# CarloLucibello/GraphNeuralNetworks.jl

Hardware: NVIDIA H100
Metric: edges/sec fwd+bwd GCNConv 128-dim on 100M-edge graph (higher is better)
Workload: dtype f32

## Files before the change

graphneuralnetworks.jl_b200/csrc/dense_tc.cu:

```cuda
#include "common.cuh"
#include <map>

namespace gnnb {

namespace tc {
constexpr int BM = 128;
constexpr int BK = 32;
constexpr int BN = 128;
constexpr int NSTAGE = 3;
constexpr int PRODUCERS = 128;
constexpr int CONSUMER_WARPS = 8;
constexpr int THREADS = PRODUCERS + CONSUMER_WARPS * 32;
constexpr int KBLK_BYTES = BM * 128;
constexpr int W_BYTES = 4 * KBLK_BYTES;
constexpr int SMEM_W_BIG = 0;
constexpr int SMEM_W_SMALL = W_BYTES;
constexpr int SMEM_A = 2 * W_BYTES;
constexpr int SMEM_BIAS = SMEM_A + NSTAGE * 2 * KBLK_BYTES;
constexpr int SMEM_BAR = SMEM_BIAS + 512;
constexpr int SMEM_TOTAL = SMEM_BAR + 64;

__device__ __forceinline__ uint32_t s_u32(const void* p) { return (uint32_t)__cvta_generic_to_shared(p); }
__device__ __forceinline__ void bar_init(uint32_t bar, uint32_t count) {
    asm volatile("mbarrier.init.shared::cta.b64 [%0], %1;" ::"r"(bar), "r"(count) : "memory");
}
__device__ __forceinline__ void bar_arrive(uint32_t bar) {
    asm volatile("mbarrier.arrive.shared::cta.b64 _, [%0];" ::"r"(bar) : "memory");
}
__device__ __forceinline__ bool bar_try(uint32_t bar, uint32_t parity) {
    uint32_t ok;
    asm volatile("{\n\t.reg .pred p;\n\tmbarrier.try_wait.parity.shared::cta.b64 p, [%1], %2;\n\tselp.u32 %0, 1, 0, p;\n\t}"
                 : "=r"(ok) : "r"(bar), "r"(parity) : "memory");
    return ok != 0;
}
__device__ __forceinline__ bool bar_wait(uint32_t bar, uint32_t parity, int* err) {
    for (uint32_t spin = 0; spin < (1u << 26); ++spin) {
        if (bar_try(bar, parity)) return true;
        if ((spin & 1023) == 1023 && *(volatile int*)err) return false;
    }
    atomicExch(err, 1);
    return false;
}
__device__ __forceinline__ float tf32_big(float x) { return __uint_as_float(__float_as_uint(x) & 0xffffe000u); }
__device__ __forceinline__ float tf32_small(float x, float b) { return isinf(x) ? 0.f : x - b; }
__device__ __forceinline__ float4 tf32_small(float4 v, float4 b) {
    return make_float4(tf32_small(v.x, b.x), tf32_small(v.y, b.y), tf32_small(v.z, b.z), tf32_small(v.w, b.w));
}
__device__ __forceinline__ void fence_proxy_async() { asm volatile("fence.proxy.async.shared::cta;" ::: "memory"); }
__device__ __forceinline__ void prefetch_l2(const void* p, uint32_t bytes) {
    asm volatile("cp.async.bulk.prefetch.L2.global [%0], %1;" ::"l"(p), "r"(bytes) : "memory");
}

__device__ __forceinline__ uint64_t gmma_desc(uint32_t saddr) {
    return (uint64_t)((saddr & 0x3ffffu) >> 4) | ((uint64_t)1 << 16) | ((uint64_t)(1024 >> 4) << 32) | ((uint64_t)1 << 62);
}
__device__ __forceinline__ void wgmma_tf32(float* d, uint64_t da, uint64_t db, uint32_t accumulate) {
    asm volatile(
        "{\n\t.reg .pred p;\n\tsetp.ne.b32 p, %66, 0;\n\t"
        "wgmma.mma_async.sync.aligned.m64n128k8.f32.tf32.tf32 "
        "{%0, %1, %2, %3, %4, %5, %6, %7, %8, %9, %10, %11, %12, %13, %14, %15, %16, %17, %18, %19, %20, %21, %22, %23, "
        "%24, %25, %26, %27, %28, %29, %30, %31, %32, %33, %34, %35, %36, %37, %38, %39, %40, %41, %42, %43, %44, %45, %46, "
        "%47, %48, %49, %50, %51, %52, %53, %54, %55, %56, %57, %58, %59, %60, %61, %62, %63}, %64, %65, p, 1, 1;\n\t}"
        : "+f"(d[0]), "+f"(d[1]), "+f"(d[2]), "+f"(d[3]), "+f"(d[4]), "+f"(d[5]), "+f"(d[6]), "+f"(d[7]), "+f"(d[8]),
          "+f"(d[9]), "+f"(d[10]), "+f"(d[11]), "+f"(d[12]), "+f"(d[13]), "+f"(d[14]), "+f"(d[15]), "+f"(d[16]),
          "+f"(d[17]), "+f"(d[18]), "+f"(d[19]), "+f"(d[20]), "+f"(d[21]), "+f"(d[22]), "+f"(d[23]), "+f"(d[24]),
          "+f"(d[25]), "+f"(d[26]), "+f"(d[27]), "+f"(d[28]), "+f"(d[29]), "+f"(d[30]), "+f"(d[31]), "+f"(d[32]),
          "+f"(d[33]), "+f"(d[34]), "+f"(d[35]), "+f"(d[36]), "+f"(d[37]), "+f"(d[38]), "+f"(d[39]), "+f"(d[40]),
          "+f"(d[41]), "+f"(d[42]), "+f"(d[43]), "+f"(d[44]), "+f"(d[45]), "+f"(d[46]), "+f"(d[47]), "+f"(d[48]),
          "+f"(d[49]), "+f"(d[50]), "+f"(d[51]), "+f"(d[52]), "+f"(d[53]), "+f"(d[54]), "+f"(d[55]), "+f"(d[56]),
          "+f"(d[57]), "+f"(d[58]), "+f"(d[59]), "+f"(d[60]), "+f"(d[61]), "+f"(d[62]), "+f"(d[63])
        : "l"(da), "l"(db), "r"(accumulate));
}
__device__ __forceinline__ void fence_acc(float* d) {
#pragma unroll
    for (int i = 0; i < 64; ++i) asm volatile("" : "+f"(d[i])::"memory");
}
__device__ __forceinline__ void wgmma_fence() { asm volatile("wgmma.fence.sync.aligned;" ::: "memory"); }
__device__ __forceinline__ void wgmma_commit() { asm volatile("wgmma.commit_group.sync.aligned;" ::: "memory"); }
__device__ __forceinline__ void wgmma_wait_all() { asm volatile("wgmma.wait_group.sync.aligned 0;" ::: "memory"); }

__device__ __forceinline__ void mma_kblock(float* dm, float* dc, uint32_t a_big, uint32_t a_small, uint32_t b_big,
                                           uint32_t b_small, bool first) {
    wgmma_fence();
    fence_acc(dm);
    fence_acc(dc);
#pragma unroll
    for (int j = 0; j < 4; ++j) {
        const uint32_t o = j * 32;
        const uint32_t acc = (first && j == 0) ? 0u : 1u;
        wgmma_tf32(dc, gmma_desc(a_small + o), gmma_desc(b_big + o), acc);
        wgmma_tf32(dc, gmma_desc(a_big + o), gmma_desc(b_small + o), 1u);
        wgmma_tf32(dm, gmma_desc(a_big + o), gmma_desc(b_big + o), dm == dc ? 1u : acc);
    }
    wgmma_commit();
    wgmma_wait_all();
    fence_acc(dm);
    fence_acc(dc);
}

struct Params {
    const float* __restrict__ x;
    const float* __restrict__ w;
    const float* __restrict__ bias;
    const float* __restrict__ addend;
    float* __restrict__ y;
    int64_t M;
    int K, Nout, relu, ldw;
    int* err;
    const float* __restrict__ wimg;
    const float* __restrict__ act;
    float* __restrict__ colsum;
    uint32_t* __restrict__ mask;
};


template <bool MASK = false>
__device__ __forceinline__ void store_tile(const Params& p, const float* dm, const float* dc, const float* sbias, int64_t row0,
                                           int col_base, int ncols) {
    const int lane = threadIdx.x & 31, w4 = (threadIdx.x >> 5) & 3;
    const int64_t r0 = row0 + w4 * 16 + (lane >> 2);
    uint32_t mw[2] = {0u, 0u};
#pragma unroll
    for (int j = 0; j < BN / 8; ++j) {
        const int c = 8 * j + 2 * (lane & 3);
        if (c >= ncols) continue;
        const float b0 = sbias[col_base + c], b1 = sbias[col_base + c + 1];
#pragma unroll
        for (int h = 0; h < 2; ++h) {
            const int64_t row = r0 + 8 * h;
            if (row >= p.M) continue;
            float2 o = make_float2((dm[4 * j + 2 * h] + dc[4 * j + 2 * h]) + b0, (dm[4 * j + 2 * h + 1] + dc[4 * j + 2 * h + 1]) + b1);
            const size_t at = (size_t)row * p.Nout + col_base + c;
            if (p.addend) {
                const float2 a = *reinterpret_cast<const float2*>(p.addend + at);
                o.x += a.x; o.y += a.y;
            }
            if (p.relu) { o.x = fmax_nan(o.x, 0.f); o.y = fmax_nan(o.y, 0.f); }
            *reinterpret_cast<float2*>(p.y + at) = o;
            if (MASK) mw[h] |= ((uint32_t)(o.x > 0.f) << (2 * j)) | ((uint32_t)(o.y > 0.f) << (2 * j + 1));
        }
    }
    if (MASK) {
#pragma unroll
        for (int h = 0; h < 2; ++h) {
            const int64_t row = r0 + 8 * h;
            if (row < p.M) p.mask[(size_t)row * 4 + (lane & 3)] = mw[h];
        }
    }
}

template <bool MASK = false>
__device__ __forceinline__ void consume_tiles(const Params& p, uint32_t sbase, const float* sbias, int KB, int64_t ntiles) {
    const int warp = threadIdx.x >> 5, lane = threadIdx.x & 31;
    const uint32_t bar_full = sbase + SMEM_BAR, bar_empty = bar_full + 8 * NSTAGE;
    const int wg = (warp - PRODUCERS / 32) >> 2;
    float dm[64] = {}, dc[64] = {};
    uint32_t it = 0;
    bool alive = true;
    for (int64_t tile = blockIdx.x; alive && tile < ntiles; tile += gridDim.x) {
        for (int kb = 0; kb < KB; ++kb, ++it) {
            const int stage = it % NSTAGE;
            if (!bar_wait(bar_full + 8 * stage, (it / NSTAGE) & 1, p.err)) { alive = false; break; }
            const uint32_t a_big = sbase + SMEM_A + stage * 2 * KBLK_BYTES + wg * 64 * 128, a_small = a_big + KBLK_BYTES;
            const uint32_t w_big = sbase + SMEM_W_BIG + kb * KBLK_BYTES, w_small = sbase + SMEM_W_SMALL + kb * KBLK_BYTES;
            mma_kblock(dm, dc, a_big, a_small, w_big, w_small, kb == 0);
            if (lane == 0) bar_arrive(bar_empty + 8 * stage);
        }
        if (alive) store_tile<MASK>(p, dm, dc, sbias, tile * BM + wg * 64, 0, p.Nout);
    }
}

template <bool MASK>
__device__ __forceinline__ void linear_body(const Params& p) {
    extern __shared__ __align__(1024) unsigned char smem[];
    const int tid = threadIdx.x, warp = tid >> 5;
    const int KB = p.K / BK;
    const int64_t ntiles = (p.M + BM - 1) / BM;
    const uint32_t sbase = s_u32(smem);
    const uint32_t bar_full = sbase + SMEM_BAR;
    const uint32_t bar_empty = bar_full + 8 * NSTAGE;
    float* sbias = reinterpret_cast<float*>(smem + SMEM_BIAS);

    if (tid == 0) {
        for (int s = 0; s < NSTAGE; ++s) { bar_init(bar_full + 8 * s, PRODUCERS); bar_init(bar_empty + 8 * s, CONSUMER_WARPS); }
        asm volatile("fence.mbarrier_init.release.cluster;" ::: "memory");
    }
    for (int i = tid; i < BN; i += THREADS) sbias[i] = (p.bias && i < p.Nout) ? p.bias[i] : 0.f;
    {
        const int kv = p.K >> 2;
        for (int idx = tid; idx < BN * kv; idx += THREADS) {
            const int n = idx / kv, c4 = idx - n * kv, kb = c4 >> 3, c = c4 & 7;
            const float4 v = n < p.Nout ? __ldg(reinterpret_cast<const float4*>(p.w + (size_t)n * p.ldw) + c4)
                                        : make_float4(0.f, 0.f, 0.f, 0.f);
            const float4 b = make_float4(tf32_big(v.x), tf32_big(v.y), tf32_big(v.z), tf32_big(v.w));
            const float4 s = tf32_small(v, b);
            const int off = kb * KBLK_BYTES + (n >> 3) * 1024 + (n & 7) * 128 + ((c ^ (n & 7)) << 4);
            *reinterpret_cast<float4*>(smem + SMEM_W_BIG + off) = b;
            *reinterpret_cast<float4*>(smem + SMEM_W_SMALL + off) = s;
        }
    }
    fence_proxy_async();
    __syncthreads();

    if (warp < PRODUCERS / 32) {
        const int c = tid & 7, r16 = tid >> 3, rr = r16 & 7;
        const int64_t my_tiles = (ntiles > (int64_t)blockIdx.x) ? (ntiles - blockIdx.x + gridDim.x - 1) / gridDim.x : 0;
        const int64_t total = my_tiles * KB;
        auto fetch = [&](int64_t item, float4* v) {
            const int64_t tile = blockIdx.x + (item / KB) * gridDim.x;
            const int kb = (int)(item % KB);
#pragma unroll
            for (int i = 0; i < 8; ++i) {
                const int64_t row = tile * BM + r16 + 16 * i;
                v[i] = (item < total && row < p.M)
                           ? __ldg(reinterpret_cast<const float4*>(p.x + (size_t)row * p.K + kb * BK) + c)
                           : make_float4(0.f, 0.f, 0.f, 0.f);
            }
        };
        float4 v[8], vn[8];
        fetch(0, v);
        for (int64_t it = 0; it < total; ++it) {
            fetch(it + 1, vn);
            const int stage = (int)(it % NSTAGE);
            if (!bar_wait(bar_empty + 8 * stage, (uint32_t)(((it / NSTAGE) & 1) ^ 1), p.err)) break;
            unsigned char* abig = smem + SMEM_A + stage * 2 * KBLK_BYTES;
#pragma unroll
            for (int i = 0; i < 8; ++i) {
                const float4 b = make_float4(tf32_big(v[i].x), tf32_big(v[i].y), tf32_big(v[i].z), tf32_big(v[i].w));
                const float4 s = tf32_small(v[i], b);
                const int off = ((r16 >> 3) + 2 * i) * 1024 + rr * 128 + ((c ^ rr) << 4);
                *reinterpret_cast<float4*>(abig + off) = b;
                *reinterpret_cast<float4*>(abig + KBLK_BYTES + off) = s;
            }
            fence_proxy_async();
            bar_arrive(bar_full + 8 * stage);
#pragma unroll
            for (int i = 0; i < 8; ++i) v[i] = vn[i];
        }
    } else {
        consume_tiles<MASK>(p, sbase, sbias, KB, ntiles);
    }
}

__global__ void __launch_bounds__(THREADS, 1) linear_tf32x3_kernel(const Params p) { linear_body<false>(p); }
__global__ void __launch_bounds__(THREADS, 1) linear_relu_mask_kernel(const Params p) { linear_body<true>(p); }

template <bool MASK>
__device__ __forceinline__ void bwd_dx_body(const Params& p) {
    extern __shared__ __align__(1024) unsigned char smem[];
    const int tid = threadIdx.x, warp = tid >> 5, lane = tid & 31;
    const int64_t ntiles = (p.M + BM - 1) / BM;
    const uint32_t sbase = s_u32(smem);
    const uint32_t bar_full = sbase + SMEM_BAR;
    const uint32_t bar_empty = bar_full + 8 * NSTAGE;
    float* sbias = reinterpret_cast<float*>(smem + SMEM_BIAS);

    if (tid == 0) {
        for (int s = 0; s < NSTAGE; ++s) { bar_init(bar_full + 8 * s, PRODUCERS); bar_init(bar_empty + 8 * s, CONSUMER_WARPS); }
        asm volatile("fence.mbarrier_init.release.cluster;" ::: "memory");
    }
    for (int i = tid; i < BN; i += THREADS) sbias[i] = 0.f;
    for (int idx = tid; idx < BN * 32; idx += THREADS) {
        const int n = idx >> 5, c4 = idx & 31, kb = c4 >> 3, c = c4 & 7;
        float4 v = make_float4(0.f, 0.f, 0.f, 0.f);
        if (n < p.Nout) {
            const float* col = p.w + (size_t)(4 * c4) * p.Nout + n;
            v = make_float4(__ldg(col), __ldg(col + p.Nout), __ldg(col + 2 * p.Nout), __ldg(col + 3 * p.Nout));
        }
        const float4 b = make_float4(tf32_big(v.x), tf32_big(v.y), tf32_big(v.z), tf32_big(v.w));
        const float4 s = tf32_small(v, b);
        const int off = kb * KBLK_BYTES + (n >> 3) * 1024 + (n & 7) * 128 + ((c ^ (n & 7)) << 4);
        *reinterpret_cast<float4*>(smem + SMEM_W_BIG + off) = b;
        *reinterpret_cast<float4*>(smem + SMEM_W_SMALL + off) = s;
    }
    fence_proxy_async();
    __syncthreads();

    if (warp < PRODUCERS / 32) {
        const int c = tid & 7, r16 = tid >> 3, rr = r16 & 7;
        const float4 zero = make_float4(0.f, 0.f, 0.f, 0.f);
        const int64_t my_tiles = (ntiles > (int64_t)blockIdx.x) ? (ntiles - blockIdx.x + gridDim.x - 1) / gridDim.x : 0;
        const int64_t total = my_tiles * 4;
        using MaskReg = typename std::conditional<MASK, uint2, float4>::type;
        auto fetch = [&](int64_t item, float4* g, MaskReg* m) {
            const int64_t tile = blockIdx.x + (item >> 2) * gridDim.x;
            const int kb = (int)(item & 3);
#pragma unroll
            for (int i = 0; i < 8; ++i) {
                const int64_t row = tile * BM + r16 + 16 * i;
                const bool in = item < total && row < p.M;
                const size_t at = (size_t)row * 128 + kb * BK;
                g[i] = in ? __ldg(reinterpret_cast<const float4*>(p.x + at) + c) : zero;
                if constexpr (MASK) m[i] = in ? __ldg(reinterpret_cast<const uint2*>(p.mask + (size_t)row * 4) + (c & 1)) : make_uint2(0u, 0u);
                else m[i] = (in && p.act) ? __ldg(reinterpret_cast<const float4*>(p.act + at) + c) : zero;
            }
        };
        auto masked = [&](float4* g, const MaskReg* m, int kb) {
            if constexpr (MASK) {
                const int s = 8 * kb + 2 * (c >> 1);
#pragma unroll
                for (int i = 0; i < 8; ++i) {
                    g[i].x = (m[i].x >> s) & 1u ? g[i].x : 0.f; g[i].y = (m[i].x >> (s + 1)) & 1u ? g[i].y : 0.f;
                    g[i].z = (m[i].y >> s) & 1u ? g[i].z : 0.f; g[i].w = (m[i].y >> (s + 1)) & 1u ? g[i].w : 0.f;
                }
            } else {
                if (!p.act) return;
#pragma unroll
                for (int i = 0; i < 8; ++i) {
                    g[i].x = m[i].x > 0.f ? g[i].x : 0.f; g[i].y = m[i].y > 0.f ? g[i].y : 0.f;
                    g[i].z = m[i].z > 0.f ? g[i].z : 0.f; g[i].w = m[i].w > 0.f ? g[i].w : 0.f;
                }
            }
        };
        float4 cs = zero;
        float4 g[8], gn[8];
        MaskReg mn[8];
        fetch(0, g, mn);
        masked(g, mn, 0);
        for (int64_t it = 0; it < total; ++it) {
            const int kb = (int)(it & 3);
            if (tid == 0 && kb == 0 && it + 4 < total) {
                const int64_t r0 = (blockIdx.x + ((it >> 2) + 1) * gridDim.x) * BM, nr = (p.M - r0 < BM) ? p.M - r0 : BM;
                prefetch_l2(p.x + (size_t)r0 * 128, (uint32_t)(nr * 512));
                if (!MASK && p.act) prefetch_l2(p.act + (size_t)r0 * 128, (uint32_t)(nr * 512));
            }
            fetch(it + 1, gn, mn);
            if (p.colsum) {
                float4 t = zero;
#pragma unroll
                for (int i = 0; i < 8; ++i) { t.x += g[i].x; t.y += g[i].y; t.z += g[i].z; t.w += g[i].w; }
#pragma unroll
                for (int o = 8; o <= 16; o <<= 1) {
                    t.x += __shfl_xor_sync(0xffffffffu, t.x, o); t.y += __shfl_xor_sync(0xffffffffu, t.y, o);
                    t.z += __shfl_xor_sync(0xffffffffu, t.z, o); t.w += __shfl_xor_sync(0xffffffffu, t.w, o);
                }
                if ((lane >> 3) == kb) { cs.x += t.x; cs.y += t.y; cs.z += t.z; cs.w += t.w; }
            }
            const int stage = (int)(it % NSTAGE);
            if (!bar_wait(bar_empty + 8 * stage, (uint32_t)(((it / NSTAGE) & 1) ^ 1), p.err)) break;
            unsigned char* abig = smem + SMEM_A + stage * 2 * KBLK_BYTES;
#pragma unroll
            for (int i = 0; i < 8; ++i) {
                const float4 b = make_float4(tf32_big(g[i].x), tf32_big(g[i].y), tf32_big(g[i].z), tf32_big(g[i].w));
                const float4 s = tf32_small(g[i], b);
                const int off = ((r16 >> 3) + 2 * i) * 1024 + rr * 128 + ((c ^ rr) << 4);
                *reinterpret_cast<float4*>(abig + off) = b;
                *reinterpret_cast<float4*>(abig + KBLK_BYTES + off) = s;
            }
            fence_proxy_async();
            bar_arrive(bar_full + 8 * stage);
#pragma unroll
            for (int i = 0; i < 8; ++i) g[i] = gn[i];
            masked(g, mn, (kb + 1) & 3);
        }
        if (p.colsum) reinterpret_cast<float4*>(p.colsum + ((size_t)blockIdx.x * 4 + warp) * 128 + (lane >> 3) * BK)[c] = cs;
    } else {
        consume_tiles(p, sbase, sbias, 128 / BK, ntiles);
    }
}

__global__ void __launch_bounds__(THREADS, 1) linear_bwd_dx_kernel(const Params p) { bwd_dx_body<false>(p); }
__global__ void __launch_bounds__(THREADS, 1) linear_bwd_dx_mask_kernel(const Params p) { bwd_dx_body<true>(p); }
}

namespace tcw {
using namespace tc;
constexpr int WSTAGE = 3;
constexpr int FLUSH = 4;
constexpr int STAGE_BYTES = 4 * KBLK_BYTES;
constexpr int SMEM_BARW = WSTAGE * STAGE_BYTES;
constexpr int SMEM_TOTALW = SMEM_BARW + 64;

struct ParamsW {
    const float* __restrict__ dpre;
    const float* __restrict__ x;
    float* __restrict__ partial;
    int64_t M, rows_per_cta;
    int Din;
    int* err;
    const float* __restrict__ act;
    const uint32_t* __restrict__ mask;
};
constexpr int L2_AHEAD = 3;

__device__ __forceinline__ int kmajor_off(int n, int k) {
    return (n >> 3) * 1024 + (n & 7) * 128 + ((((k >> 2) ^ (n & 7))) << 4) + (k & 3) * 4;
}

template <bool FUSED, bool MASK = false>
__device__ __forceinline__ void dw_body(const ParamsW& p) {
    extern __shared__ __align__(1024) unsigned char smem[];
    const int tid = threadIdx.x, warp = tid >> 5, lane = tid & 31;
    const uint32_t sbase = s_u32(smem);
    const uint32_t bar_full = sbase + SMEM_BARW, bar_empty = bar_full + 8 * WSTAGE;
    const int nfB = p.Din >> 2;
    const int64_t r_begin = (int64_t)blockIdx.x * p.rows_per_cta;
    const int64_t r_end = (r_begin + p.rows_per_cta < p.M) ? r_begin + p.rows_per_cta : p.M;
    const int64_t nblk = (r_end > r_begin) ? (r_end - r_begin + 31) / 32 : 0;

    if (tid == 0) {
        for (int s = 0; s < WSTAGE; ++s) { bar_init(bar_full + 8 * s, PRODUCERS); bar_init(bar_empty + 8 * s, CONSUMER_WARPS); }
        asm volatile("fence.mbarrier_init.release.cluster;" ::: "memory");
    }
    for (int i = tid; i < SMEM_BARW / 16; i += THREADS) reinterpret_cast<float4*>(smem)[i] = make_float4(0.f, 0.f, 0.f, 0.f);
    fence_proxy_async();
    __syncthreads();

    if (warp < PRODUCERS / 32) {
        const int rl = lane >> 2, fl = lane & 3;
        auto load = [&](const float* src, int ld, int nf, int64_t blk, float4* v) {
#pragma unroll
            for (int q = 0; q < 8; ++q) {
                const int64_t r = r_begin + blk * 32 + rl + 8 * (q & 3);
                const int f = 4 * (warp + 4 * (q >> 2)) + fl;
                v[q] = (blk < nblk && r < r_end && f < nf) ? __ldg(reinterpret_cast<const float4*>(src + (size_t)r * ld) + f)
                                                           : make_float4(0.f, 0.f, 0.f, 0.f);
            }
        };
        auto put1 = [&](unsigned char* big, int n, int k, float e) {
            const int off = kmajor_off(n, k);
            const float b = tf32_big(e);
            *reinterpret_cast<float*>(big + off) = b;
            *reinterpret_cast<float*>(big + KBLK_BYTES + off) = tf32_small(e, b);
        };
        auto put = [&](unsigned char* big, int n0, int k, float4 v) {
            put1(big, n0, k, v.x); put1(big, n0 + 1, k, v.y); put1(big, n0 + 2, k, v.z); put1(big, n0 + 3, k, v.w);
        };
        auto stage_in = [&](int64_t blk, const float4* va, const float4* vb) {
            const int stage = (int)(blk % WSTAGE);
            if (!bar_wait(bar_empty + 8 * stage, (uint32_t)(((blk / WSTAGE) & 1) ^ 1), p.err)) return false;
            unsigned char* st = smem + stage * STAGE_BYTES;
#pragma unroll
            for (int q = 0; q < 8; ++q) {
                const int k = rl + 8 * (q & 3);
                const int f = 4 * (warp + 4 * (q >> 2)) + fl;
                put(st, 4 * f, k, va[q]);
                if (f < nfB) put(st + 2 * KBLK_BYTES, 4 * f, k, vb[q]);
            }
            fence_proxy_async();
            bar_arrive(bar_full + 8 * stage);
            return true;
        };
        if constexpr (!FUSED) {
            float4 va[8], vb[8], na[8], nb[8];
            load(p.dpre, 128, 32, 0, va);
            load(p.x, p.Din, nfB, 0, vb);
            for (int64_t blk = 0; blk < nblk; ++blk) {
                load(p.dpre, 128, 32, blk + 1, na);
                load(p.x, p.Din, nfB, blk + 1, nb);
                if (!stage_in(blk, va, vb)) break;
#pragma unroll
                for (int q = 0; q < 8; ++q) { va[q] = na[q]; vb[q] = nb[q]; }
            }
        } else if constexpr (MASK) {
            float4 va[8], vb[8], na[8];
            uint2 nm[4];
            auto load_mask = [&](int64_t blk) {
#pragma unroll
                for (int q = 0; q < 4; ++q) {
                    const int64_t r = r_begin + blk * 32 + rl + 8 * q;
                    nm[q] = (blk < nblk && r < r_end) ? __ldg(reinterpret_cast<const uint2*>(p.mask + (size_t)r * 4) + (fl & 1))
                                                      : make_uint2(0u, 0u);
                }
            };
            auto promote = [&]() {
#pragma unroll
                for (int q = 0; q < 8; ++q) {
                    const uint2 m = nm[q & 3];
                    const int s = 4 * (warp + 4 * (q >> 2)) + 2 * (fl >> 1);
                    va[q].x = (m.x >> s) & 1u ? na[q].x : 0.f; va[q].y = (m.x >> (s + 1)) & 1u ? na[q].y : 0.f;
                    va[q].z = (m.y >> s) & 1u ? na[q].z : 0.f; va[q].w = (m.y >> (s + 1)) & 1u ? na[q].w : 0.f;
                }
            };
            load(p.dpre, 128, 32, 0, na);
            load_mask(0);
            promote();
            for (int64_t blk = 0; blk < nblk; ++blk) {
                if (tid == 0 && blk + L2_AHEAD < nblk) {
                    const int64_t ra = r_begin + 32 * (blk + L2_AHEAD), nr = (r_end - ra < 32) ? r_end - ra : 32;
                    prefetch_l2(p.dpre + (size_t)ra * 128, (uint32_t)(nr * 512));
                    prefetch_l2(p.x + (size_t)ra * p.Din, (uint32_t)(nr * p.Din * 4));
                }
                load(p.dpre, 128, 32, blk + 1, na);
                load_mask(blk + 1);
                load(p.x, p.Din, nfB, blk, vb);
                if (!stage_in(blk, va, vb)) break;
                promote();
            }
        } else {
            float4 va[8], vb[8], na[8], nm[8];
            auto promote = [&]() {
#pragma unroll
                for (int q = 0; q < 8; ++q) {
                    va[q] = na[q];
                    if (p.act) {
                        va[q].x = nm[q].x > 0.f ? va[q].x : 0.f; va[q].y = nm[q].y > 0.f ? va[q].y : 0.f;
                        va[q].z = nm[q].z > 0.f ? va[q].z : 0.f; va[q].w = nm[q].w > 0.f ? va[q].w : 0.f;
                    }
                }
            };
            load(p.dpre, 128, 32, 0, na);
            if (p.act) load(p.act, 128, 32, 0, nm);
            promote();
            for (int64_t blk = 0; blk < nblk; ++blk) {
                if (tid == 0 && blk + L2_AHEAD < nblk) {
                    const int64_t ra = r_begin + 32 * (blk + L2_AHEAD), nr = (r_end - ra < 32) ? r_end - ra : 32;
                    prefetch_l2(p.dpre + (size_t)ra * 128, (uint32_t)(nr * 512));
                    if (p.act) prefetch_l2(p.act + (size_t)ra * 128, (uint32_t)(nr * 512));
                    prefetch_l2(p.x + (size_t)ra * p.Din, (uint32_t)(nr * p.Din * 4));
                }
                load(p.dpre, 128, 32, blk + 1, na);
                if (p.act) load(p.act, 128, 32, blk + 1, nm);
                load(p.x, p.Din, nfB, blk, vb);
                if (!stage_in(blk, va, vb)) break;
                promote();
            }
        }
    } else {
        const int wg = (warp - PRODUCERS / 32) >> 2;
        float acc[64] = {}, sum[64];
#pragma unroll
        for (int i = 0; i < 64; ++i) sum[i] = 0.f;
        for (int64_t blk = 0; blk < nblk; ++blk) {
            const int stage = (int)(blk % WSTAGE);
            if (!bar_wait(bar_full + 8 * stage, (uint32_t)((blk / WSTAGE) & 1), p.err)) break;
            const uint32_t a_big = sbase + stage * STAGE_BYTES + wg * 64 * 128, a_small = a_big + KBLK_BYTES;
            const uint32_t b_big = sbase + stage * STAGE_BYTES + 2 * KBLK_BYTES, b_small = b_big + KBLK_BYTES;
            mma_kblock(acc, acc, a_big, a_small, b_big, b_small, (blk % FLUSH) == 0);
            if (lane == 0) bar_arrive(bar_empty + 8 * stage);
            if ((blk % FLUSH) == FLUSH - 1 || blk == nblk - 1) {
#pragma unroll
                for (int i = 0; i < 64; ++i) sum[i] += acc[i];
            }
        }
        const int w4 = warp & 3;
        const int i0 = wg * 64 + w4 * 16 + (lane >> 2);
#pragma unroll
        for (int j = 0; j < BN / 8; ++j) {
            const int c = 8 * j + 2 * (lane & 3);
            if (c >= p.Din) continue;
#pragma unroll
            for (int h = 0; h < 2; ++h) {
                float* prow = p.partial + ((size_t)blockIdx.x * 128 + i0 + 8 * h) * p.Din;
                *reinterpret_cast<float2*>(prow + c) = make_float2(sum[4 * j + 2 * h], sum[4 * j + 2 * h + 1]);
            }
        }
    }
}

__global__ void __launch_bounds__(THREADS, 1) dw_tf32x3_kernel(const ParamsW p) { dw_body<false>(p); }
__global__ void __launch_bounds__(THREADS, 1) linear_bwd_dw_kernel(const ParamsW p) { dw_body<true>(p); }
__global__ void __launch_bounds__(THREADS, 1) linear_bwd_dw_mask_kernel(const ParamsW p) { dw_body<true, true>(p); }

__global__ void dw_reduce_kernel(const float* __restrict__ partial, int nparts, int n, float* __restrict__ dW,
                                 const float* __restrict__ colsum = nullptr, int ncolsum = 0, float* __restrict__ db = nullptr) {
    const int i = blockIdx.x * blockDim.x + threadIdx.x;
    if (i < n) {
        float acc = 0.f;
        for (int b = 0; b < nparts; ++b) acc += partial[(size_t)b * n + i];
        dW[i] = acc;
    } else if (db && i < n + 128) {
        float acc = 0.f;
        for (int b = 0; b < ncolsum; ++b) acc += colsum[(size_t)b * 128 + i - n];
        db[i - n] = acc;
    }
}
}

namespace tcx {
using namespace tc;
constexpr int XSTAGE = 3;
constexpr int XSTAGE_BYTES = 4 * KBLK_BYTES;
constexpr int SMEM_BIAS_X = XSTAGE * XSTAGE_BYTES;
constexpr int MAX_NOUT = 1024;
constexpr int SMEM_BAR_X = SMEM_BIAS_X + MAX_NOUT * 4;
constexpr int SMEM_TOTAL_X = SMEM_BAR_X + 64;

__global__ void w_image_kernel(const float* __restrict__ w, int ldw, int K, int Nout, float* __restrict__ wimg) {
    const int kv = K >> 2, KB = K / BK;
    const int idx = blockIdx.x * blockDim.x + threadIdx.x;
    if (idx >= Nout * kv) return;
    const int n = idx / kv, c4 = idx - n * kv, kb = c4 >> 3, c = c4 & 7;
    const int nq = n >> 7, nl = n & 127;
    const float4 v = __ldg(reinterpret_cast<const float4*>(w + (size_t)n * ldw) + c4);
    const float4 b = make_float4(tf32_big(v.x), tf32_big(v.y), tf32_big(v.z), tf32_big(v.w));
    const float4 sm = tf32_small(v, b);
    unsigned char* blk = reinterpret_cast<unsigned char*>(wimg) + (size_t)(nq * KB + kb) * (2 * KBLK_BYTES);
    const int off = (nl >> 3) * 1024 + (nl & 7) * 128 + ((c ^ (nl & 7)) << 4);
    *reinterpret_cast<float4*>(blk + off) = b;
    *reinterpret_cast<float4*>(blk + KBLK_BYTES + off) = sm;
}

__device__ __forceinline__ void bulk_g2s(uint32_t dst, const void* src, uint32_t bytes, uint32_t bar) {
    asm volatile("cp.async.bulk.shared::cluster.global.mbarrier::complete_tx::bytes [%0], [%1], %2, [%3];"
                 ::"r"(dst), "l"(src), "r"(bytes), "r"(bar) : "memory");
}
__device__ __forceinline__ void bar_expect_tx(uint32_t bar, uint32_t bytes) {
    asm volatile("mbarrier.arrive.expect_tx.shared::cta.b64 _, [%0], %1;" ::"r"(bar), "r"(bytes) : "memory");
}

__global__ void __launch_bounds__(THREADS, 1) linear_wide_tf32x3_kernel(const Params p) {
    extern __shared__ __align__(1024) unsigned char smem[];
    const int tid = threadIdx.x, warp = tid >> 5, lane = tid & 31;
    const int KB = p.K / BK;
    const int NQ = p.Nout / 128;
    const int64_t ntiles = (p.M + BM - 1) / BM;
    const int64_t my_tiles = (ntiles > (int64_t)blockIdx.x) ? (ntiles - blockIdx.x + gridDim.x - 1) / gridDim.x : 0;
    const uint32_t sbase = s_u32(smem);
    const uint32_t bar_full = sbase + SMEM_BAR_X;
    const uint32_t bar_empty = bar_full + 8 * XSTAGE;
    float* sbias = reinterpret_cast<float*>(smem + SMEM_BIAS_X);

    if (tid == 0) {
        for (int s = 0; s < XSTAGE; ++s) { bar_init(bar_full + 8 * s, PRODUCERS + 1); bar_init(bar_empty + 8 * s, CONSUMER_WARPS); }
        asm volatile("fence.mbarrier_init.release.cluster;" ::: "memory");
    }
    for (int i = tid; i < p.Nout; i += THREADS) sbias[i] = p.bias ? p.bias[i] : 0.f;
    __syncthreads();

    if (warp < PRODUCERS / 32) {
        const int c = tid & 7, r16 = tid >> 3, rr = r16 & 7;
        const int64_t total = my_tiles * NQ * KB;
        int64_t f_tile = blockIdx.x;
        int f_nq = 0, f_kb = 0;
        auto fetch = [&](int64_t item, float4* va) {
#pragma unroll
            for (int i = 0; i < 8; ++i) {
                const int64_t row = f_tile * BM + r16 + 16 * i;
                va[i] = (item < total && row < p.M)
                            ? __ldg(reinterpret_cast<const float4*>(p.x + (size_t)row * p.K + f_kb * BK) + c)
                            : make_float4(0.f, 0.f, 0.f, 0.f);
            }
            if (++f_kb == KB) { f_kb = 0; if (++f_nq == NQ) { f_nq = 0; f_tile += gridDim.x; } }
        };
        float4 va[8], na[8], na2[8];
        fetch(0, va);
        fetch(1, na);
        int w_blk = 0;
        const int w_blocks = NQ * KB;
        for (int64_t it = 0; it < total; ++it) {
            fetch(it + 2, na2);
            const int stage = (int)(it % XSTAGE);
            if (!bar_wait(bar_empty + 8 * stage, (uint32_t)(((it / XSTAGE) & 1) ^ 1), p.err)) break;
            unsigned char* sa = smem + stage * XSTAGE_BYTES;
            if (tid == 0) {
                bar_expect_tx(bar_full + 8 * stage, 2 * KBLK_BYTES);
                bulk_g2s(sbase + stage * XSTAGE_BYTES + 2 * KBLK_BYTES,
                         reinterpret_cast<const unsigned char*>(p.wimg) + (size_t)w_blk * (2 * KBLK_BYTES), 2 * KBLK_BYTES,
                         bar_full + 8 * stage);
            }
            if (++w_blk == w_blocks) w_blk = 0;
#pragma unroll
            for (int i = 0; i < 8; ++i) {
                const int off = ((r16 >> 3) + 2 * i) * 1024 + rr * 128 + ((c ^ rr) << 4);
                const float4 b = make_float4(tf32_big(va[i].x), tf32_big(va[i].y), tf32_big(va[i].z), tf32_big(va[i].w));
                *reinterpret_cast<float4*>(sa + off) = b;
                *reinterpret_cast<float4*>(sa + KBLK_BYTES + off) = tf32_small(va[i], b);
            }
            fence_proxy_async();
            bar_arrive(bar_full + 8 * stage);
#pragma unroll
            for (int i = 0; i < 8; ++i) { va[i] = na[i]; na[i] = na2[i]; }
        }
    } else {
        const int wg = (warp - PRODUCERS / 32) >> 2;
        float dm[64] = {}, dc[64] = {};
        uint32_t it = 0;
        for (int64_t t = 0; t < my_tiles; ++t) {
            const int64_t tile = blockIdx.x + t * gridDim.x;
            for (int nq = 0; nq < NQ; ++nq) {
                for (int kb = 0; kb < KB; ++kb, ++it) {
                    const int stage = it % XSTAGE;
                    if (!bar_wait(bar_full + 8 * stage, (it / XSTAGE) & 1, p.err)) return;
                    const uint32_t a_big = sbase + stage * XSTAGE_BYTES + wg * 64 * 128, a_small = a_big + KBLK_BYTES;
                    const uint32_t w_big = sbase + stage * XSTAGE_BYTES + 2 * KBLK_BYTES, w_small = w_big + KBLK_BYTES;
                    mma_kblock(dm, dc, a_big, a_small, w_big, w_small, kb == 0);
                    if (lane == 0) bar_arrive(bar_empty + 8 * stage);
                }
                store_tile(p, dm, dc, sbias, tile * BM + wg * 64, nq * 128, 128);
            }
        }
    }
}
}

int g_tc_enabled = 1;

static std::mutex g_states_mu;
static std::map<int, DeviceState> g_states;

int device_state(DeviceState** out) {
    int dev = 0;
    GNNB_CUDA(cudaGetDevice(&dev));
    std::lock_guard<std::mutex> lock(g_states_mu);
    auto it = g_states.find(dev);
    if (it == g_states.end()) {
        GNNB_CUDA(cudaFuncSetAttribute(tc::linear_tf32x3_kernel, cudaFuncAttributeMaxDynamicSharedMemorySize, tc::SMEM_TOTAL));
        GNNB_CUDA(cudaFuncSetAttribute(tc::linear_relu_mask_kernel, cudaFuncAttributeMaxDynamicSharedMemorySize, tc::SMEM_TOTAL));
        GNNB_CUDA(cudaFuncSetAttribute(tcx::linear_wide_tf32x3_kernel, cudaFuncAttributeMaxDynamicSharedMemorySize, tcx::SMEM_TOTAL_X));
        GNNB_CUDA(cudaFuncSetAttribute(tcw::dw_tf32x3_kernel, cudaFuncAttributeMaxDynamicSharedMemorySize, tcw::SMEM_TOTALW));
        GNNB_CUDA(cudaFuncSetAttribute(tc::linear_bwd_dx_kernel, cudaFuncAttributeMaxDynamicSharedMemorySize, tc::SMEM_TOTAL));
        GNNB_CUDA(cudaFuncSetAttribute(tcw::linear_bwd_dw_kernel, cudaFuncAttributeMaxDynamicSharedMemorySize, tcw::SMEM_TOTALW));
        GNNB_CUDA(cudaFuncSetAttribute(tc::linear_bwd_dx_mask_kernel, cudaFuncAttributeMaxDynamicSharedMemorySize, tc::SMEM_TOTAL));
        GNNB_CUDA(cudaFuncSetAttribute(tcw::linear_bwd_dw_mask_kernel, cudaFuncAttributeMaxDynamicSharedMemorySize, tcw::SMEM_TOTALW));
        DeviceState s;
        GNNB_CUDA(cudaDeviceGetAttribute(&s.nsm, cudaDevAttrMultiProcessorCount, dev));
        DeviceScratch sc;
        GNNB_TRY(sc.alloc(&s.tc_err, 1));
        GNNB_CUDA(cudaMemset(s.tc_err, 0, sizeof(int)));
        sc.release(s.tc_err);
        it = g_states.emplace(dev, s).first;
    }
    *out = &it->second;
    return GNNB_OK;
}

int linear_tf32x3_ex(const float* x, const float* W, int64_t ldw, const float* bias, const float* addend, int relu, int64_t M,
                     int64_t K, int64_t Nout, float* y, cudaStream_t st);
int linear_tf32x3(const float* x, const float* W, const float* bias, int relu, int64_t M, int64_t K, int64_t Nout, float* y,
                  cudaStream_t st) {
    return linear_tf32x3_ex(x, W, K, bias, nullptr, relu, M, K, Nout, y, st);
}
static int linear_launch(const float* x, const float* W, int64_t ldw, const float* bias, const float* addend, int relu,
                         int64_t M, int64_t K, int64_t Nout, float* y, uint32_t* mask, cudaStream_t st);
int linear_tf32x3_ex(const float* x, const float* W, int64_t ldw, const float* bias, const float* addend, int relu, int64_t M,
                     int64_t K, int64_t Nout, float* y, cudaStream_t st) {
    return linear_launch(x, W, ldw, bias, addend, relu, M, K, Nout, y, nullptr, st);
}
int linear_relu_mask_tf32x3(const float* x, const float* W, const float* bias, int64_t M, int64_t K, float* y, uint32_t* mask,
                            cudaStream_t st) {
    if (K % 32 != 0 || K < 32 || K > 128 || ((uintptr_t)mask & 15)) return GNNB_EUNSUPPORTED;
    return linear_launch(x, W, K, bias, nullptr, 1, M, K, 128, y, mask, st);
}
static int linear_launch(const float* x, const float* W, int64_t ldw, const float* bias, const float* addend, int relu,
                         int64_t M, int64_t K, int64_t Nout, float* y, uint32_t* mask, cudaStream_t st) {
    if (!g_tc_enabled) return GNNB_EUNSUPPORTED;
    const bool wide = K > 128 || Nout > 128;
    if (wide) {
        if (K % 32 != 0 || K > 2048 || Nout % 128 != 0 || Nout > tcx::MAX_NOUT || ldw % 4 != 0 || ldw < K || M < 2048) return GNNB_EUNSUPPORTED;
    } else if (K % 32 != 0 || Nout % 16 != 0 || Nout < 16 || ldw % 4 != 0 || ldw < K) {
        return GNNB_EUNSUPPORTED;
    }
    if (((uintptr_t)x & 15) || ((uintptr_t)W & 15) || ((uintptr_t)y & 15) || ((uintptr_t)addend & 15)) return GNNB_EUNSUPPORTED;
    if (M == 0) return GNNB_OK;
    DeviceState* s = nullptr;
    GNNB_TRY(device_state(&s));
    tc::Params p;
    p.x = x; p.w = W; p.bias = bias; p.addend = addend; p.y = y; p.M = M; p.K = (int)K; p.Nout = (int)Nout; p.relu = relu;
    p.ldw = (int)ldw; p.err = s->tc_err; p.wimg = nullptr; p.act = nullptr; p.colsum = nullptr; p.mask = mask;
    if (wide) {
        GNNB_TRY(grow_buffer(&s->wimg, &s->wimg_bytes, sizeof(float) * (size_t)2 * K * Nout));
        tcx::w_image_kernel<<<(unsigned)ceil_div(Nout * (K / 4), 256), 256, 0, st>>>(W, (int)ldw, (int)K, (int)Nout, s->wimg);
        GNNB_LAUNCHED();
        p.wimg = s->wimg;
    }
    const int nsm = s->nsm;
    const int64_t ntiles = ceil_div(M, tc::BM);
    const unsigned grid = (unsigned)(ntiles < nsm ? ntiles : nsm);
    if (wide) tcx::linear_wide_tf32x3_kernel<<<grid, tc::THREADS, tcx::SMEM_TOTAL_X, st>>>(p);
    else if (mask) tc::linear_relu_mask_kernel<<<grid, tc::THREADS, tc::SMEM_TOTAL, st>>>(p);
    else tc::linear_tf32x3_kernel<<<grid, tc::THREADS, tc::SMEM_TOTAL, st>>>(p);
    GNNB_LAUNCHED();
    return GNNB_OK;
}

int dw_tf32x3(const float* dpre, const float* x, int64_t M, int64_t Din, int64_t Dout, float* dW, cudaStream_t st) {
    if (!g_tc_enabled) return GNNB_EUNSUPPORTED;
    if (Dout != 128 || Din % 32 != 0 || Din > 128 || Din < 32) return GNNB_EUNSUPPORTED;
    if (((uintptr_t)dpre & 15) || ((uintptr_t)x & 15) || ((uintptr_t)dW & 15)) return GNNB_EUNSUPPORTED;
    DeviceState* s = nullptr;
    GNNB_TRY(device_state(&s));
    const int nsm = s->nsm;
    GNNB_TRY(grow_buffer(&s->dw_part, &s->dw_part_bytes, sizeof(float) * (size_t)nsm * 128 * 128));
    float* partial = s->dw_part;
    if (M == 0) { GNNB_CUDA(cudaMemsetAsync(dW, 0, sizeof(float) * (size_t)(Dout * Din), st)); return GNNB_OK; }
    tcw::ParamsW p;
    p.dpre = dpre; p.x = x; p.partial = partial; p.M = M; p.Din = (int)Din; p.err = s->tc_err; p.act = nullptr; p.mask = nullptr;
    int64_t rpc = ceil_div(M, nsm);
    rpc = ceil_div(rpc, 32) * 32;
    p.rows_per_cta = rpc;
    const int grid = (int)ceil_div(M, rpc);
    tcw::dw_tf32x3_kernel<<<grid, tc::THREADS, tcw::SMEM_TOTALW, st>>>(p);
    GNNB_LAUNCHED();
    const int n = (int)(128 * Din);
    tcw::dw_reduce_kernel<<<(unsigned)ceil_div(n, 256), 256, 0, st>>>(partial, grid, n, dW);
    GNNB_LAUNCHED();
    return GNNB_OK;
}

int linear_bwd_tf32x3(const float* dy, const float* y, const uint32_t* mask, const float* x, const float* W, int64_t M,
                      int64_t Din, float* dx, float* dW, float* db, cudaStream_t st) {
    if (!g_tc_enabled) return GNNB_EUNSUPPORTED;
    if (Din % 32 != 0 || Din > 128 || Din < 32 || M <= 0) return GNNB_EUNSUPPORTED;
    if (((uintptr_t)dy & 15) || ((uintptr_t)y & 15) || ((uintptr_t)x & 15) || ((uintptr_t)dx & 15) || ((uintptr_t)mask & 15))
        return GNNB_EUNSUPPORTED;
    DeviceState* s = nullptr;
    GNNB_TRY(device_state(&s));
    const int nsm = s->nsm;
    GNNB_TRY(grow_buffer(&s->bwd_part, &s->bwd_part_bytes, sizeof(float) * (size_t)nsm * 128 * 128));
    GNNB_TRY(grow_buffer(&s->bwd_colsum, &s->bwd_colsum_bytes, sizeof(float) * (size_t)nsm * 4 * 128));
    float *partial = s->bwd_part, *colsum = s->bwd_colsum;
    tc::Params p;
    p.x = dy; p.w = W; p.bias = nullptr; p.addend = nullptr; p.y = dx; p.M = M; p.K = 128; p.Nout = (int)Din; p.relu = 0;
    p.ldw = 128; p.err = s->tc_err; p.wimg = nullptr; p.act = y; p.colsum = db ? colsum : nullptr;
    p.mask = const_cast<uint32_t*>(mask);
    const int64_t ntiles = ceil_div(M, tc::BM);
    const int grid_dx = (int)(ntiles < nsm ? ntiles : nsm);
    if (mask) tc::linear_bwd_dx_mask_kernel<<<grid_dx, tc::THREADS, tc::SMEM_TOTAL, st>>>(p);
    else tc::linear_bwd_dx_kernel<<<grid_dx, tc::THREADS, tc::SMEM_TOTAL, st>>>(p);
    GNNB_LAUNCHED();
    tcw::ParamsW pw;
    pw.dpre = dy; pw.x = x; pw.partial = partial; pw.M = M; pw.Din = (int)Din; pw.err = s->tc_err; pw.act = y; pw.mask = mask;
    const int64_t rpc = ceil_div(ceil_div(M, nsm), 32) * 32;
    pw.rows_per_cta = rpc;
    const int grid_dw = (int)ceil_div(M, rpc);
    if (mask) tcw::linear_bwd_dw_mask_kernel<<<grid_dw, tc::THREADS, tcw::SMEM_TOTALW, st>>>(pw);
    else tcw::linear_bwd_dw_kernel<<<grid_dw, tc::THREADS, tcw::SMEM_TOTALW, st>>>(pw);
    GNNB_LAUNCHED();
    const int n = (int)(128 * Din);
    tcw::dw_reduce_kernel<<<(unsigned)ceil_div(n + 128, 256), 256, 0, st>>>(partial, grid_dw, n, dW, colsum, grid_dx * 4, db);
    GNNB_LAUNCHED();
    return GNNB_OK;
}

int linear_tf32x3_error() {
    std::lock_guard<std::mutex> lock(g_states_mu);
    for (const auto& kv : g_states) {
        int e = 0;
        cudaMemcpy(&e, kv.second.tc_err, sizeof(int), cudaMemcpyDeviceToHost);
        if (e) return e;
    }
    return 0;
}

}
```

graphneuralnetworks.jl_b200/csrc/tma.cuh:

```cuda
#pragma once
#include <cuda_runtime.h>
#include <stdint.h>

namespace gnnb {
namespace tma {

__device__ __forceinline__ uint32_t smem_u32(const void* p) { return (uint32_t)__cvta_generic_to_shared(p); }
__device__ __forceinline__ void mbar_init(uint32_t bar, uint32_t count) {
    asm volatile("mbarrier.init.shared::cta.b64 [%0], %1;" ::"r"(bar), "r"(count) : "memory");
}
__device__ __forceinline__ void mbar_expect_tx(uint32_t bar, uint32_t bytes) {
    asm volatile("mbarrier.arrive.expect_tx.shared::cta.b64 _, [%0], %1;" ::"r"(bar), "r"(bytes) : "memory");
}
__device__ __forceinline__ bool mbar_try(uint32_t bar, uint32_t parity) {
    uint32_t ok;
    asm volatile("{\n\t.reg .pred p;\n\tmbarrier.try_wait.parity.shared::cta.b64 p, [%1], %2;\n\tselp.u32 %0, 1, 0, p;\n\t}"
                 : "=r"(ok) : "r"(bar), "r"(parity) : "memory");
    return ok != 0;
}
__device__ __forceinline__ bool mbar_wait_bounded(uint32_t bar, uint32_t parity, int* err) {
    for (uint32_t spin = 0; spin < (1u << 26); ++spin) {
        if (mbar_try(bar, parity)) return true;
        if ((spin & 1023) == 1023 && *(volatile int*)err) return false;
    }
    atomicExch(err, 1);
    return false;
}
__device__ __forceinline__ void fence_proxy_async() { asm volatile("fence.proxy.async.shared::cta;" ::: "memory"); }
__device__ __forceinline__ void bulk_load(uint32_t dst, const void* src, uint32_t bytes, uint32_t bar) {
    asm volatile("cp.async.bulk.shared::cluster.global.mbarrier::complete_tx::bytes [%0], [%1], %2, [%3];"
                 ::"r"(dst), "l"(src), "r"(bytes), "r"(bar) : "memory");
}

}
}
```

Measured before the change: 2.279 billion.

## Feed TF32x3 dense kernels through a TMA ring with register-sourced WGMMA

Replaces the 128-thread producer that loaded, split into big and small TF32 parts and stored tiles to shared memory with a single-thread TMA tensor-map loader feeding a deeper ring of up to six stages. Consumers now read the raw fp32 tile from shared memory, apply the mask or activation gating, split into big and small parts in registers, and issue register-sourced WGMMA with one group kept in flight. setmaxnreg moves registers from producers to consumers. The aim is to cut producer load and store traffic and overlap MMA with the next stage, at the cost of consumer-side conversion work and host-side tensor-map encoding on every launch.

```diff
diff --git a/graphneuralnetworks.jl_b200/csrc/dense_tc.cu b/graphneuralnetworks.jl_b200/csrc/dense_tc.cu
--- a/graphneuralnetworks.jl_b200/csrc/dense_tc.cu
+++ b/graphneuralnetworks.jl_b200/csrc/dense_tc.cu
@@ -1,4 +1,6 @@
 #include "common.cuh"
+#include "tma.cuh"
+#include <cudaTypedefs.h>
 #include <map>
 
 namespace gnnb {
@@ -7,7 +9,6 @@
 constexpr int BM = 128;
 constexpr int BK = 32;
 constexpr int BN = 128;
-constexpr int NSTAGE = 3;
 constexpr int PRODUCERS = 128;
 constexpr int CONSUMER_WARPS = 8;
 constexpr int THREADS = PRODUCERS + CONSUMER_WARPS * 32;
@@ -16,9 +17,16 @@
 constexpr int SMEM_W_BIG = 0;
 constexpr int SMEM_W_SMALL = W_BYTES;
 constexpr int SMEM_A = 2 * W_BYTES;
-constexpr int SMEM_BIAS = SMEM_A + NSTAGE * 2 * KBLK_BYTES;
+constexpr int RING_BYTES = 6 * KBLK_BYTES;
+constexpr int MAX_STAGES = 6;
+constexpr int MASK_BYTES = BM * 16;
+constexpr int SMEM_BIAS = SMEM_A + RING_BYTES;
 constexpr int SMEM_BAR = SMEM_BIAS + 512;
-constexpr int SMEM_TOTAL = SMEM_BAR + 64;
+constexpr int SMEM_TOTAL = SMEM_BAR + 16 * MAX_STAGES;
+constexpr int PRODUCER_REGS = 56;
+constexpr int CONSUMER_REGS = 224;
+static_assert(SMEM_TOTAL <= 227 * 1024, "shared memory of the ring kernels");
+static_assert(PRODUCERS * PRODUCER_REGS + CONSUMER_WARPS * 32 * CONSUMER_REGS <= 65536, "register split");
 
 __device__ __forceinline__ uint32_t s_u32(const void* p) { return (uint32_t)__cvta_generic_to_shared(p); }
 __device__ __forceinline__ void bar_init(uint32_t bar, uint32_t count) {
@@ -47,9 +55,6 @@
     return make_float4(tf32_small(v.x, b.x), tf32_small(v.y, b.y), tf32_small(v.z, b.z), tf32_small(v.w, b.w));
 }
 __device__ __forceinline__ void fence_proxy_async() { asm volatile("fence.proxy.async.shared::cta;" ::: "memory"); }
-__device__ __forceinline__ void prefetch_l2(const void* p, uint32_t bytes) {
-    asm volatile("cp.async.bulk.prefetch.L2.global [%0], %1;" ::"l"(p), "r"(bytes) : "memory");
-}
 
 __device__ __forceinline__ uint64_t gmma_desc(uint32_t saddr) {
     return (uint64_t)((saddr & 0x3ffffu) >> 4) | ((uint64_t)1 << 16) | ((uint64_t)(1024 >> 4) << 32) | ((uint64_t)1 << 62);
@@ -98,6 +103,39 @@
     fence_acc(dc);
 }
 
+__device__ __forceinline__ void wgmma_tf32_rs(float* d, const uint32_t* a, uint64_t db, uint32_t accumulate) {
+    asm volatile(
+        "{\n\t.reg .pred p;\n\tsetp.ne.b32 p, %69, 0;\n\t"
+        "wgmma.mma_async.sync.aligned.m64n128k8.f32.tf32.tf32 "
+        "{%0, %1, %2, %3, %4, %5, %6, %7, %8, %9, %10, %11, %12, %13, %14, %15, %16, %17, %18, %19, %20, %21, %22, %23, "
+        "%24, %25, %26, %27, %28, %29, %30, %31, %32, %33, %34, %35, %36, %37, %38, %39, %40, %41, %42, %43, %44, %45, %46, "
+        "%47, %48, %49, %50, %51, %52, %53, %54, %55, %56, %57, %58, %59, %60, %61, %62, %63}, {%64, %65, %66, %67}, %68, p, 1, 1;\n\t}"
+        : "+f"(d[0]), "+f"(d[1]), "+f"(d[2]), "+f"(d[3]), "+f"(d[4]), "+f"(d[5]), "+f"(d[6]), "+f"(d[7]), "+f"(d[8]),
+          "+f"(d[9]), "+f"(d[10]), "+f"(d[11]), "+f"(d[12]), "+f"(d[13]), "+f"(d[14]), "+f"(d[15]), "+f"(d[16]),
+          "+f"(d[17]), "+f"(d[18]), "+f"(d[19]), "+f"(d[20]), "+f"(d[21]), "+f"(d[22]), "+f"(d[23]), "+f"(d[24]),
+          "+f"(d[25]), "+f"(d[26]), "+f"(d[27]), "+f"(d[28]), "+f"(d[29]), "+f"(d[30]), "+f"(d[31]), "+f"(d[32]),
+          "+f"(d[33]), "+f"(d[34]), "+f"(d[35]), "+f"(d[36]), "+f"(d[37]), "+f"(d[38]), "+f"(d[39]), "+f"(d[40]),
+          "+f"(d[41]), "+f"(d[42]), "+f"(d[43]), "+f"(d[44]), "+f"(d[45]), "+f"(d[46]), "+f"(d[47]), "+f"(d[48]),
+          "+f"(d[49]), "+f"(d[50]), "+f"(d[51]), "+f"(d[52]), "+f"(d[53]), "+f"(d[54]), "+f"(d[55]), "+f"(d[56]),
+          "+f"(d[57]), "+f"(d[58]), "+f"(d[59]), "+f"(d[60]), "+f"(d[61]), "+f"(d[62]), "+f"(d[63])
+        : "r"(a[0]), "r"(a[1]), "r"(a[2]), "r"(a[3]), "l"(db), "r"(accumulate));
+}
+__device__ __forceinline__ void wgmma_wait_1() { asm volatile("wgmma.wait_group.sync.aligned 1;" ::: "memory"); }
+
+__device__ __forceinline__ void mma_kblock_rs(float* dm, float* dc, const uint32_t* ab, const uint32_t* as, uint32_t b_big,
+                                              uint32_t b_small, bool first) {
+    wgmma_fence();
+#pragma unroll
+    for (int j = 0; j < 4; ++j) {
+        const uint32_t o = j * 32;
+        const uint32_t acc = (first && j == 0) ? 0u : 1u;
+        wgmma_tf32_rs(dc, as + 4 * j, gmma_desc(b_big + o), acc);
+        wgmma_tf32_rs(dc, ab + 4 * j, gmma_desc(b_small + o), 1u);
+        wgmma_tf32_rs(dm, ab + 4 * j, gmma_desc(b_big + o), dm == dc ? 1u : acc);
+    }
+    wgmma_commit();
+}
+
 struct Params {
     const float* __restrict__ x;
     const float* __restrict__ w;
@@ -149,43 +187,102 @@
     }
 }
 
-template <bool MASK = false>
-__device__ __forceinline__ void consume_tiles(const Params& p, uint32_t sbase, const float* sbias, int KB, int64_t ntiles) {
+__host__ __device__ constexpr int ring_stage_bytes(int boxes, bool mask) { return boxes * KBLK_BYTES + (mask ? MASK_BYTES : 0); }
+__host__ __device__ constexpr int ring_stages(int stage_bytes) {
+    return RING_BYTES / stage_bytes < MAX_STAGES ? RING_BYTES / stage_bytes : MAX_STAGES;
+}
+
+template <bool MASK_OUT, int DPRE>
+__device__ __forceinline__ void consume_ring(const Params& p, unsigned char* smem, const float* sbias, int KB, int64_t ntiles,
+                                             int ns, int stage_bytes) {
     const int warp = threadIdx.x >> 5, lane = threadIdx.x & 31;
-    const uint32_t bar_full = sbase + SMEM_BAR, bar_empty = bar_full + 8 * NSTAGE;
-    const int wg = (warp - PRODUCERS / 32) >> 2;
+    const int wg = (warp - PRODUCERS / 32) >> 2, g = lane >> 2, t = lane & 3;
+    const int r0 = wg * 64 + (warp & 3) * 16 + g;
+    const uint32_t sbase = s_u32(smem);
+    const uint32_t bar_full = sbase + SMEM_BAR, bar_empty = bar_full + 8 * MAX_STAGES;
+    const int64_t my_tiles = (ntiles > (int64_t)blockIdx.x) ? (ntiles - blockIdx.x + gridDim.x - 1) / gridDim.x : 0;
+    const int64_t total = my_tiles * KB;
     float dm[64] = {}, dc[64] = {};
-    uint32_t it = 0;
+    uint32_t ab0[16], as0[16], ab1[16], as1[16];
+    int stage = 0, kb = 0;
+    uint32_t phase = 0;
+    int64_t tile = blockIdx.x;
     bool alive = true;
-    for (int64_t tile = blockIdx.x; alive && tile < ntiles; tile += gridDim.x) {
-        for (int kb = 0; kb < KB; ++kb, ++it) {
-            const int stage = it % NSTAGE;
-            if (!bar_wait(bar_full + 8 * stage, (it / NSTAGE) & 1, p.err)) { alive = false; break; }
-            const uint32_t a_big = sbase + SMEM_A + stage * 2 * KBLK_BYTES + wg * 64 * 128, a_small = a_big + KBLK_BYTES;
-            const uint32_t w_big = sbase + SMEM_W_BIG + kb * KBLK_BYTES, w_small = sbase + SMEM_W_SMALL + kb * KBLK_BYTES;
-            mma_kblock(dm, dc, a_big, a_small, w_big, w_small, kb == 0);
-            if (lane == 0) bar_arrive(bar_empty + 8 * stage);
-        }
-        if (alive) store_tile<MASK>(p, dm, dc, sbias, tile * BM + wg * 64, 0, p.Nout);
+    auto step = [&](uint32_t* ab, uint32_t* as) {
+        if (!bar_wait(bar_full + 8 * stage, phase, p.err)) { alive = false; return; }
+        const unsigned char* st = smem + SMEM_A + stage * stage_bytes;
+        uint32_t mw[4];
+        if constexpr (DPRE == 1) {
+            const uint32_t* m = reinterpret_cast<const uint32_t*>(st + KBLK_BYTES) + (t >> 1);
+#pragma unroll
+            for (int e = 0; e < 4; ++e) mw[e] = m[(r0 + 8 * (e & 1)) * 4 + 2 * (e >> 1)];
+        }
+#pragma unroll
+        for (int j = 0; j < 4; ++j) {
+#pragma unroll
+            for (int e = 0; e < 4; ++e) {
+                const int off = (r0 + 8 * (e & 1)) * 128 + (((2 * j + (e >> 1)) ^ g) << 4) + 4 * t;
+                float v = *reinterpret_cast<const float*>(st + off);
+                if constexpr (DPRE == 1) v = (mw[e] >> (8 * kb + 2 * j + (t & 1))) & 1u ? v : 0.f;
+                if constexpr (DPRE == 2) {
+                    if (p.act) v = *reinterpret_cast<const float*>(st + KBLK_BYTES + off) > 0.f ? v : 0.f;
+                }
+                const float b = tf32_big(v);
+                ab[4 * j + e] = __float_as_uint(b);
+                as[4 * j + e] = __float_as_uint(tf32_small(v, b));
+            }
+        }
+        __syncwarp();
+        if (lane == 0) bar_arrive(bar_empty + 8 * stage);
+        fence_acc(dm);
+        fence_acc(dc);
+        mma_kblock_rs(dm, dc, ab, as, sbase + SMEM_W_BIG + kb * KBLK_BYTES, sbase + SMEM_W_SMALL + kb * KBLK_BYTES, kb == 0);
+        wgmma_wait_1();
+        if (++stage == ns) { stage = 0; phase ^= 1; }
+        if (++kb == KB) {
+            wgmma_wait_all();
+            fence_acc(dm);
+            fence_acc(dc);
+            store_tile<MASK_OUT>(p, dm, dc, sbias, tile * BM + wg * 64, 0, p.Nout);
+            kb = 0;
+            tile += gridDim.x;
+        }
+    };
+    for (int64_t it = 0; alive && it < total; it += 2) {
+        step(ab0, as0);
+        if (alive && it + 1 < total) step(ab1, as1);
+    }
+    wgmma_wait_all();
+}
+
+__device__ __forceinline__ void ring_init(unsigned char* smem, const float* bias, int nbias, int readers) {
+    const int tid = threadIdx.x;
+    if (tid == 0) {
+        const uint32_t bar_full = s_u32(smem + SMEM_BAR), bar_empty = bar_full + 8 * MAX_STAGES;
+        for (int s = 0; s < MAX_STAGES; ++s) { bar_init(bar_full + 8 * s, 1); bar_init(bar_empty + 8 * s, readers); }
+        asm volatile("fence.mbarrier_init.release.cluster;" ::: "memory");
+    }
+    float* sbias = reinterpret_cast<float*>(smem + SMEM_BIAS);
+    for (int i = tid; i < BN; i += THREADS) sbias[i] = (bias && i < nbias) ? bias[i] : 0.f;
+}
+
+__device__ __forceinline__ void ring_drain(uint32_t bar_full, int ns, int stage, uint32_t phase, int64_t issued) {
+    for (int k = 0; k < ns && k < issued; ++k) {
+        if (--stage < 0) { stage = ns - 1; phase ^= 1; }
+        for (uint32_t spin = 0; spin < (1u << 22) && !bar_try(bar_full + 8 * stage, phase); ++spin) {}
     }
 }
 
 template <bool MASK>
-__device__ __forceinline__ void linear_body(const Params& p) {
+__device__ __forceinline__ void linear_body(const Params& p, const CUtensorMap* tm_x) {
     extern __shared__ __align__(1024) unsigned char smem[];
     const int tid = threadIdx.x, warp = tid >> 5;
     const int KB = p.K / BK;
     const int64_t ntiles = (p.M + BM - 1) / BM;
     const uint32_t sbase = s_u32(smem);
-    const uint32_t bar_full = sbase + SMEM_BAR;
-    const uint32_t bar_empty = bar_full + 8 * NSTAGE;
-    float* sbias = reinterpret_cast<float*>(smem + SMEM_BIAS);
-
-    if (tid == 0) {
-        for (int s = 0; s < NSTAGE; ++s) { bar_init(bar_full + 8 * s, PRODUCERS); bar_init(bar_empty + 8 * s, CONSUMER_WARPS); }
-        asm volatile("fence.mbarrier_init.release.cluster;" ::: "memory");
-    }
-    for (int i = tid; i < BN; i += THREADS) sbias[i] = (p.bias && i < p.Nout) ? p.bias[i] : 0.f;
+    constexpr int stage_bytes = ring_stage_bytes(1, false), ns = ring_stages(stage_bytes);
+
+    ring_init(smem, p.bias, p.Nout, CONSUMER_WARPS);
     {
         const int kv = p.K >> 2;
         for (int idx = tid; idx < BN * kv; idx += THREADS) {
@@ -203,63 +300,44 @@
     __syncthreads();
 
     if (warp < PRODUCERS / 32) {
-        const int c = tid & 7, r16 = tid >> 3, rr = r16 & 7;
+        asm volatile("setmaxnreg.dec.sync.aligned.u32 %0;" ::"n"(PRODUCER_REGS));
+        if (tid != 0) return;
+        const uint32_t bar_full = sbase + SMEM_BAR, bar_empty = bar_full + 8 * MAX_STAGES;
         const int64_t my_tiles = (ntiles > (int64_t)blockIdx.x) ? (ntiles - blockIdx.x + gridDim.x - 1) / gridDim.x : 0;
-        const int64_t total = my_tiles * KB;
-        auto fetch = [&](int64_t item, float4* v) {
-            const int64_t tile = blockIdx.x + (item / KB) * gridDim.x;
-            const int kb = (int)(item % KB);
-#pragma unroll
-            for (int i = 0; i < 8; ++i) {
-                const int64_t row = tile * BM + r16 + 16 * i;
-                v[i] = (item < total && row < p.M)
-                           ? __ldg(reinterpret_cast<const float4*>(p.x + (size_t)row * p.K + kb * BK) + c)
-                           : make_float4(0.f, 0.f, 0.f, 0.f);
-            }
-        };
-        float4 v[8], vn[8];
-        fetch(0, v);
-        for (int64_t it = 0; it < total; ++it) {
-            fetch(it + 1, vn);
-            const int stage = (int)(it % NSTAGE);
-            if (!bar_wait(bar_empty + 8 * stage, (uint32_t)(((it / NSTAGE) & 1) ^ 1), p.err)) break;
-            unsigned char* abig = smem + SMEM_A + stage * 2 * KBLK_BYTES;
-#pragma unroll
-            for (int i = 0; i < 8; ++i) {
-                const float4 b = make_float4(tf32_big(v[i].x), tf32_big(v[i].y), tf32_big(v[i].z), tf32_big(v[i].w));
-                const float4 s = tf32_small(v[i], b);
-                const int off = ((r16 >> 3) + 2 * i) * 1024 + rr * 128 + ((c ^ rr) << 4);
-                *reinterpret_cast<float4*>(abig + off) = b;
-                *reinterpret_cast<float4*>(abig + KBLK_BYTES + off) = s;
-            }
-            fence_proxy_async();
-            bar_arrive(bar_full + 8 * stage);
-#pragma unroll
-            for (int i = 0; i < 8; ++i) v[i] = vn[i];
-        }
+        int stage = 0, kb = 0;
+        uint32_t phase = 0;
+        int64_t tile = blockIdx.x, it = 0;
+        for (; it < my_tiles * KB; ++it) {
+            if (!bar_wait(bar_empty + 8 * stage, phase ^ 1, p.err)) break;
+            tma::mbar_expect_tx(bar_full + 8 * stage, KBLK_BYTES);
+            tma::tensor_load_2d(sbase + SMEM_A + stage * stage_bytes, tm_x, kb * BK, (int)(tile * BM), bar_full + 8 * stage);
+            if (++stage == ns) { stage = 0; phase ^= 1; }
+            if (++kb == KB) { kb = 0; tile += gridDim.x; }
+        }
+        ring_drain(bar_full, ns, stage, phase, it);
     } else {
-        consume_tiles<MASK>(p, sbase, sbias, KB, ntiles);
-    }
-}
-
-__global__ void __launch_bounds__(THREADS, 1) linear_tf32x3_kernel(const Params p) { linear_body<false>(p); }
-__global__ void __launch_bounds__(THREADS, 1) linear_relu_mask_kernel(const Params p) { linear_body<true>(p); }
+        asm volatile("setmaxnreg.inc.sync.aligned.u32 %0;" ::"n"(CONSUMER_REGS));
+        consume_ring<MASK, 0>(p, smem, reinterpret_cast<float*>(smem + SMEM_BIAS), KB, ntiles, ns, stage_bytes);
+    }
+}
+
+__global__ void __launch_bounds__(THREADS, 1) linear_tf32x3_kernel(const Params p, const __grid_constant__ CUtensorMap tm_x) {
+    linear_body<false>(p, &tm_x);
+}
+__global__ void __launch_bounds__(THREADS, 1) linear_relu_mask_kernel(const Params p, const __grid_constant__ CUtensorMap tm_x) {
+    linear_body<true>(p, &tm_x);
+}
 
 template <bool MASK>
-__device__ __forceinline__ void bwd_dx_body(const Params& p) {
+__device__ __forceinline__ void bwd_dx_body(const Params& p, const CUtensorMap* tm_dy, const CUtensorMap* tm_y) {
     extern __shared__ __align__(1024) unsigned char smem[];
     const int tid = threadIdx.x, warp = tid >> 5, lane = tid & 31;
     const int64_t ntiles = (p.M + BM - 1) / BM;
     const uint32_t sbase = s_u32(smem);
-    const uint32_t bar_full = sbase + SMEM_BAR;
-    const uint32_t bar_empty = bar_full + 8 * NSTAGE;
-    float* sbias = reinterpret_cast<float*>(smem + SMEM_BIAS);
-
-    if (tid == 0) {
-        for (int s = 0; s < NSTAGE; ++s) { bar_init(bar_full + 8 * s, PRODUCERS); bar_init(bar_empty + 8 * s, CONSUMER_WARPS); }
-        asm volatile("fence.mbarrier_init.release.cluster;" ::: "memory");
-    }
-    for (int i = tid; i < BN; i += THREADS) sbias[i] = 0.f;
+    const int boxes = (!MASK && p.act) ? 2 : 1;
+    const int stage_bytes = ring_stage_bytes(boxes, MASK), ns = ring_stages(stage_bytes);
+
+    ring_init(smem, nullptr, 0, CONSUMER_WARPS + PRODUCERS / 32);
     for (int idx = tid; idx < BN * 32; idx += THREADS) {
         const int n = idx >> 5, c4 = idx & 31, kb = c4 >> 3, c = c4 & 7;
         float4 v = make_float4(0.f, 0.f, 0.f, 0.f);
@@ -277,99 +355,97 @@
     __syncthreads();
 
     if (warp < PRODUCERS / 32) {
+        asm volatile("setmaxnreg.dec.sync.aligned.u32 %0;" ::"n"(PRODUCER_REGS));
+        const uint32_t bar_full = sbase + SMEM_BAR, bar_empty = bar_full + 8 * MAX_STAGES;
         const int c = tid & 7, r16 = tid >> 3, rr = r16 & 7;
-        const float4 zero = make_float4(0.f, 0.f, 0.f, 0.f);
         const int64_t my_tiles = (ntiles > (int64_t)blockIdx.x) ? (ntiles - blockIdx.x + gridDim.x - 1) / gridDim.x : 0;
         const int64_t total = my_tiles * 4;
-        using MaskReg = typename std::conditional<MASK, uint2, float4>::type;
-        auto fetch = [&](int64_t item, float4* g, MaskReg* m) {
-            const int64_t tile = blockIdx.x + (item >> 2) * gridDim.x;
-            const int kb = (int)(item & 3);
-#pragma unroll
-            for (int i = 0; i < 8; ++i) {
-                const int64_t row = tile * BM + r16 + 16 * i;
-                const bool in = item < total && row < p.M;
-                const size_t at = (size_t)row * 128 + kb * BK;
-                g[i] = in ? __ldg(reinterpret_cast<const float4*>(p.x + at) + c) : zero;
-                if constexpr (MASK) m[i] = in ? __ldg(reinterpret_cast<const uint2*>(p.mask + (size_t)row * 4) + (c & 1)) : make_uint2(0u, 0u);
-                else m[i] = (in && p.act) ? __ldg(reinterpret_cast<const float4*>(p.act + at) + c) : zero;
-            }
+        int i_stage = 0, i_kb = 0;
+        uint32_t i_phase = 0;
+        int64_t i_tile = blockIdx.x;
+        bool issuing = true;
+        auto issue = [&]() {
+            if (!issuing) return;
+            if (!bar_wait(bar_empty + 8 * i_stage, i_phase ^ 1, p.err)) { issuing = false; return; }
+            {
+                const uint32_t dst = sbase + SMEM_A + i_stage * stage_bytes, full = bar_full + 8 * i_stage;
+                const int64_t nr = (p.M - i_tile * BM < BM) ? p.M - i_tile * BM : BM;
+                tma::mbar_expect_tx(full, boxes * KBLK_BYTES + (MASK ? (uint32_t)nr * 16 : 0u));
+                tma::tensor_load_2d(dst, tm_dy, i_kb * BK, (int)(i_tile * BM), full);
+                if (boxes == 2) tma::tensor_load_2d(dst + KBLK_BYTES, tm_y, i_kb * BK, (int)(i_tile * BM), full);
+                if (MASK) tma::bulk_load(dst + KBLK_BYTES, p.mask + (size_t)i_tile * BM * 4, (uint32_t)nr * 16, full);
+            }
+            if (++i_stage == ns) { i_stage = 0; i_phase ^= 1; }
+            if (++i_kb == 4) { i_kb = 0; i_tile += gridDim.x; }
         };
-        auto masked = [&](float4* g, const MaskReg* m, int kb) {
-            if constexpr (MASK) {
-                const int s = 8 * kb + 2 * (c >> 1);
-#pragma unroll
-                for (int i = 0; i < 8; ++i) {
-                    g[i].x = (m[i].x >> s) & 1u ? g[i].x : 0.f; g[i].y = (m[i].x >> (s + 1)) & 1u ? g[i].y : 0.f;
-                    g[i].z = (m[i].y >> s) & 1u ? g[i].z : 0.f; g[i].w = (m[i].y >> (s + 1)) & 1u ? g[i].w : 0.f;
-                }
-            } else {
-                if (!p.act) return;
-#pragma unroll
-                for (int i = 0; i < 8; ++i) {
-                    g[i].x = m[i].x > 0.f ? g[i].x : 0.f; g[i].y = m[i].y > 0.f ? g[i].y : 0.f;
-                    g[i].z = m[i].z > 0.f ? g[i].z : 0.f; g[i].w = m[i].w > 0.f ? g[i].w : 0.f;
-                }
-            }
-        };
+        if (tid == 0)
+            for (int64_t n = 0; n < ns - 1 && n < total; ++n) issue();
+        const float4 zero = make_float4(0.f, 0.f, 0.f, 0.f);
         float4 cs = zero;
-        float4 g[8], gn[8];
-        MaskReg mn[8];
-        fetch(0, g, mn);
-        masked(g, mn, 0);
+        int stage = 0;
+        uint32_t phase = 0;
         for (int64_t it = 0; it < total; ++it) {
             const int kb = (int)(it & 3);
-            if (tid == 0 && kb == 0 && it + 4 < total) {
-                const int64_t r0 = (blockIdx.x + ((it >> 2) + 1) * gridDim.x) * BM, nr = (p.M - r0 < BM) ? p.M - r0 : BM;
-                prefetch_l2(p.x + (size_t)r0 * 128, (uint32_t)(nr * 512));
-                if (!MASK && p.act) prefetch_l2(p.act + (size_t)r0 * 128, (uint32_t)(nr * 512));
-            }
-            fetch(it + 1, gn, mn);
+            if (tid == 0 && it + ns - 1 < total) issue();
+            if (!bar_wait(bar_full + 8 * stage, phase, p.err)) break;
             if (p.colsum) {
-                float4 t = zero;
-#pragma unroll
-                for (int i = 0; i < 8; ++i) { t.x += g[i].x; t.y += g[i].y; t.z += g[i].z; t.w += g[i].w; }
+                const unsigned char* st = smem + SMEM_A + stage * stage_bytes;
+                float4 s = zero;
+#pragma unroll
+                for (int i = 0; i < 8; ++i) {
+                    const int off = ((r16 >> 3) + 2 * i) * 1024 + rr * 128 + ((c ^ rr) << 4);
+                    float4 g = *reinterpret_cast<const float4*>(st + off);
+                    if constexpr (MASK) {
+                        const uint2 m = *reinterpret_cast<const uint2*>(st + KBLK_BYTES + (r16 + 16 * i) * 16 + (c & 1) * 8);
+                        const int sh = 8 * kb + 2 * (c >> 1);
+                        g.x = (m.x >> sh) & 1u ? g.x : 0.f; g.y = (m.x >> (sh + 1)) & 1u ? g.y : 0.f;
+                        g.z = (m.y >> sh) & 1u ? g.z : 0.f; g.w = (m.y >> (sh + 1)) & 1u ? g.w : 0.f;
+                    } else if (boxes == 2) {
+                        const float4 m = *reinterpret_cast<const float4*>(st + KBLK_BYTES + off);
+                        g.x = m.x > 0.f ? g.x : 0.f; g.y = m.y > 0.f ? g.y : 0.f;
+                        g.z = m.z > 0.f ? g.z : 0.f; g.w = m.w > 0.f ? g.w : 0.f;
+                    }
+                    s.x += g.x; s.y += g.y; s.z += g.z; s.w += g.w;
+                }
 #pragma unroll
                 for (int o = 8; o <= 16; o <<= 1) {
-                    t.x += __shfl_xor_sync(0xffffffffu, t.x, o); t.y += __shfl_xor_sync(0xffffffffu, t.y, o);
-                    t.z += __shfl_xor_sync(0xffffffffu, t.z, o); t.w += __shfl_xor_sync(0xffffffffu, t.w, o);
+                    s.x += __shfl_xor_sync(0xffffffffu, s.x, o); s.y += __shfl_xor_sync(0xffffffffu, s.y, o);
+                    s.z += __shfl_xor_sync(0xffffffffu, s.z, o); s.w += __shfl_xor_sync(0xffffffffu, s.w, o);
                 }
-                if ((lane >> 3) == kb) { cs.x += t.x; cs.y += t.y; cs.z += t.z; cs.w += t.w; }
-            }
-            const int stage = (int)(it % NSTAGE);
-            if (!bar_wait(bar_empty + 8 * stage, (uint32_t)(((it / NSTAGE) & 1) ^ 1), p.err)) break;
-            unsigned char* abig = smem + SMEM_A + stage * 2 * KBLK_BYTES;
-#pragma unroll
-            for (int i = 0; i < 8; ++i) {
-                const float4 b = make_float4(tf32_big(g[i].x), tf32_big(g[i].y), tf32_big(g[i].z), tf32_big(g[i].w));
-                const float4 s = tf32_small(g[i], b);
-                const int off = ((r16 >> 3) + 2 * i) * 1024 + rr * 128 + ((c ^ rr) << 4);
-                *reinterpret_cast<float4*>(abig + off) = b;
-                *reinterpret_cast<float4*>(abig + KBLK_BYTES + off) = s;
-            }
-            fence_proxy_async();
-            bar_arrive(bar_full + 8 * stage);
-#pragma unroll
-            for (int i = 0; i < 8; ++i) g[i] = gn[i];
-            masked(g, mn, (kb + 1) & 3);
-        }
+                if ((lane >> 3) == kb) { cs.x += s.x; cs.y += s.y; cs.z += s.z; cs.w += s.w; }
+            }
+            __syncwarp();
+            if (lane == 0) bar_arrive(bar_empty + 8 * stage);
+            if (++stage == ns) { stage = 0; phase ^= 1; }
+        }
+        if (tid == 0) ring_drain(bar_full, ns, i_stage, i_phase, (i_tile - blockIdx.x) / gridDim.x * 4 + i_kb);
         if (p.colsum) reinterpret_cast<float4*>(p.colsum + ((size_t)blockIdx.x * 4 + warp) * 128 + (lane >> 3) * BK)[c] = cs;
     } else {
-        consume_tiles(p, sbase, sbias, 128 / BK, ntiles);
-    }
-}
-
-__global__ void __launch_bounds__(THREADS, 1) linear_bwd_dx_kernel(const Params p) { bwd_dx_body<false>(p); }
-__global__ void __launch_bounds__(THREADS, 1) linear_bwd_dx_mask_kernel(const Params p) { bwd_dx_body<true>(p); }
+        asm volatile("setmaxnreg.inc.sync.aligned.u32 %0;" ::"n"(CONSUMER_REGS));
+        consume_ring<false, MASK ? 1 : 2>(p, smem, reinterpret_cast<float*>(smem + SMEM_BIAS), 128 / BK, ntiles, ns, stage_bytes);
+    }
+}
+
+__global__ void __launch_bounds__(THREADS, 1) linear_bwd_dx_kernel(const Params p, const __grid_constant__ CUtensorMap tm_dy,
+                                                                   const __grid_constant__ CUtensorMap tm_y) {
+    bwd_dx_body<false>(p, &tm_dy, &tm_y);
+}
+__global__ void __launch_bounds__(THREADS, 1) linear_bwd_dx_mask_kernel(const Params p, const __grid_constant__ CUtensorMap tm_dy,
+                                                                        const __grid_constant__ CUtensorMap tm_y) {
+    bwd_dx_body<true>(p, &tm_dy, &tm_y);
+}
 }
 
 namespace tcw {
 using namespace tc;
-constexpr int WSTAGE = 3;
 constexpr int FLUSH = 4;
-constexpr int STAGE_BYTES = 4 * KBLK_BYTES;
-constexpr int SMEM_BARW = WSTAGE * STAGE_BYTES;
-constexpr int SMEM_TOTALW = SMEM_BARW + 64;
+constexpr int BOX_BYTES = 32 * 128;
+constexpr int RINGW_BYTES = 160 * 1024;
+constexpr int MAX_WSTAGES = 4;
+constexpr int SMEM_BIMG = RINGW_BYTES;
+constexpr int SMEM_BARW = SMEM_BIMG + 4 * KBLK_BYTES;
+constexpr int SMEM_TOTALW = SMEM_BARW + 8 * (2 * MAX_WSTAGES + 4);
+static_assert(SMEM_TOTALW <= 227 * 1024, "shared memory of the dW kernels");
 
 struct ParamsW {
     const float* __restrict__ dpre;
@@ -381,176 +457,175 @@
     const float* __restrict__ act;
     const uint32_t* __restrict__ mask;
 };
-constexpr int L2_AHEAD = 3;
 
 __device__ __forceinline__ int kmajor_off(int n, int k) {
     return (n >> 3) * 1024 + (n & 7) * 128 + ((((k >> 2) ^ (n & 7))) << 4) + (k & 3) * 4;
 }
-
-template <bool FUSED, bool MASK = false>
-__device__ __forceinline__ void dw_body(const ParamsW& p) {
+__device__ __forceinline__ int box_off(int r, int c) {
+    return (c >> 5) * BOX_BYTES + r * 128 + ((((c & 31) >> 2) ^ (r & 7)) << 4) + (c & 3) * 4;
+}
+
+template <int DPRE>
+__device__ __forceinline__ void dw_body(const ParamsW& p, const CUtensorMap* tm_dy, const CUtensorMap* tm_y,
+                                        const CUtensorMap* tm_x) {
     extern __shared__ __align__(1024) unsigned char smem[];
     const int tid = threadIdx.x, warp = tid >> 5, lane = tid & 31;
     const uint32_t sbase = s_u32(smem);
-    const uint32_t bar_full = sbase + SMEM_BARW, bar_empty = bar_full + 8 * WSTAGE;
-    const int nfB = p.Din >> 2;
+    const uint32_t bar_full = sbase + SMEM_BARW, bar_empty = bar_full + 8 * MAX_WSTAGES;
+    const uint32_t bar_bfull = bar_empty + 8 * MAX_WSTAGES, bar_bempty = bar_bfull + 16;
+    const bool with_y = DPRE == 2 && p.act;
+    const int x_at = (with_y ? 8 : 4) * BOX_BYTES, mask_at = x_at + 4 * BOX_BYTES;
+    const int stage_bytes = mask_at + 1024, ns = RINGW_BYTES / stage_bytes < MAX_WSTAGES ? RINGW_BYTES / stage_bytes : MAX_WSTAGES;
+    const int xboxes = p.Din >> 5;
     const int64_t r_begin = (int64_t)blockIdx.x * p.rows_per_cta;
     const int64_t r_end = (r_begin + p.rows_per_cta < p.M) ? r_begin + p.rows_per_cta : p.M;
     const int64_t nblk = (r_end > r_begin) ? (r_end - r_begin + 31) / 32 : 0;
 
     if (tid == 0) {
-        for (int s = 0; s < WSTAGE; ++s) { bar_init(bar_full + 8 * s, PRODUCERS); bar_init(bar_empty + 8 * s, CONSUMER_WARPS); }
+        for (int s = 0; s < MAX_WSTAGES; ++s) { bar_init(bar_full + 8 * s, 1); bar_init(bar_empty + 8 * s, CONSUMER_WARPS + 4); }
+        for (int s = 0; s < 2; ++s) { bar_init(bar_bfull + 8 * s, 4); bar_init(bar_bempty + 8 * s, CONSUMER_WARPS); }
         asm volatile("fence.mbarrier_init.release.cluster;" ::: "memory");
     }
-    for (int i = tid; i < SMEM_BARW / 16; i += THREADS) reinterpret_cast<float4*>(smem)[i] = make_float4(0.f, 0.f, 0.f, 0.f);
+    for (int i = tid; i < 4 * KBLK_BYTES / 16; i += THREADS)
+        reinterpret_cast<float4*>(smem + SMEM_BIMG)[i] = make_float4(0.f, 0.f, 0.f, 0.f);
     fence_proxy_async();
     __syncthreads();
 
     if (warp < PRODUCERS / 32) {
-        const int rl = lane >> 2, fl = lane & 3;
-        auto load = [&](const float* src, int ld, int nf, int64_t blk, float4* v) {
-#pragma unroll
-            for (int q = 0; q < 8; ++q) {
-                const int64_t r = r_begin + blk * 32 + rl + 8 * (q & 3);
-                const int f = 4 * (warp + 4 * (q >> 2)) + fl;
-                v[q] = (blk < nblk && r < r_end && f < nf) ? __ldg(reinterpret_cast<const float4*>(src + (size_t)r * ld) + f)
-                                                           : make_float4(0.f, 0.f, 0.f, 0.f);
-            }
+        asm volatile("setmaxnreg.dec.sync.aligned.u32 %0;" ::"n"(PRODUCER_REGS));
+        int i_stage = 0;
+        uint32_t i_phase = 0;
+        int64_t i_blk = 0;
+        bool issuing = true;
+        auto issue = [&]() {
+            if (!issuing) return;
+            if (!bar_wait(bar_empty + 8 * i_stage, i_phase ^ 1, p.err)) { issuing = false; return; }
+            {
+                const uint32_t dst = sbase + i_stage * stage_bytes, full = bar_full + 8 * i_stage;
+                const int64_t r0 = r_begin + 32 * i_blk;
+                const uint32_t nr = (uint32_t)((r_end - r0 < 32) ? r_end - r0 : 32);
+                tma::mbar_expect_tx(full, (uint32_t)(((with_y ? 8 : 4) + xboxes) * BOX_BYTES) + (DPRE == 1 ? nr * 16 : 0u));
+                for (int b = 0; b < 4; ++b) tma::tensor_load_2d(dst + b * BOX_BYTES, tm_dy, 32 * b, (int)r0, full);
+                if (with_y)
+                    for (int b = 0; b < 4; ++b) tma::tensor_load_2d(dst + (4 + b) * BOX_BYTES, tm_y, 32 * b, (int)r0, full);
+                for (int b = 0; b < xboxes; ++b) tma::tensor_load_2d(dst + x_at + b * BOX_BYTES, tm_x, 32 * b, (int)r0, full);
+                if (DPRE == 1) tma::bulk_load(dst + mask_at, p.mask + (size_t)r0 * 4, nr * 16, full);
+            }
+            if (++i_stage == ns) { i_stage = 0; i_phase ^= 1; }
+            ++i_blk;
         };
-        auto put1 = [&](unsigned char* big, int n, int k, float e) {
-            const int off = kmajor_off(n, k);
-            const float b = tf32_big(e);
-            *reinterpret_cast<float*>(big + off) = b;
-            *reinterpret_cast<float*>(big + KBLK_BYTES + off) = tf32_small(e, b);
-        };
-        auto put = [&](unsigned char* big, int n0, int k, float4 v) {
-            put1(big, n0, k, v.x); put1(big, n0 + 1, k, v.y); put1(big, n0 + 2, k, v.z); put1(big, n0 + 3, k, v.w);
-        };
-        auto stage_in = [&](int64_t blk, const float4* va, const float4* vb) {
-            const int stage = (int)(blk % WSTAGE);
-            if (!bar_wait(bar_empty + 8 * stage, (uint32_t)(((blk / WSTAGE) & 1) ^ 1), p.err)) return false;
-            unsigned char* st = smem + stage * STAGE_BYTES;
-#pragma unroll
-            for (int q = 0; q < 8; ++q) {
-                const int k = rl + 8 * (q & 3);
-                const int f = 4 * (warp + 4 * (q >> 2)) + fl;
-                put(st, 4 * f, k, va[q]);
-                if (f < nfB) put(st + 2 * KBLK_BYTES, 4 * f, k, vb[q]);
+        if (tid == 0)
+            for (int64_t n = 0; n < ns - 1 && n < nblk; ++n) issue();
+        int stage = 0;
+        uint32_t phase = 0;
+        for (int64_t blk = 0; blk < nblk; ++blk) {
+            if (tid == 0 && blk + ns - 1 < nblk) issue();
+            const int slot = (int)(blk & 1);
+            if (!bar_wait(bar_full + 8 * stage, phase, p.err)) break;
+            if (!bar_wait(bar_bempty + 8 * slot, (uint32_t)(((blk >> 1) & 1) ^ 1), p.err)) break;
+            const unsigned char* sx = smem + stage * stage_bytes + x_at;
+            unsigned char* big = smem + SMEM_BIMG + slot * 2 * KBLK_BYTES;
+            for (int item = warp; item < xboxes * 8; item += 4) {
+                const int j = 32 * (item >> 3) + lane, q = item & 7;
+                float4 v;
+                v.x = *reinterpret_cast<const float*>(sx + box_off(4 * q, j));
+                v.y = *reinterpret_cast<const float*>(sx + box_off(4 * q + 1, j));
+                v.z = *reinterpret_cast<const float*>(sx + box_off(4 * q + 2, j));
+                v.w = *reinterpret_cast<const float*>(sx + box_off(4 * q + 3, j));
+                const float4 b = make_float4(tf32_big(v.x), tf32_big(v.y), tf32_big(v.z), tf32_big(v.w));
+                const int off = kmajor_off(j, 4 * q);
+                *reinterpret_cast<float4*>(big + off) = b;
+                *reinterpret_cast<float4*>(big + KBLK_BYTES + off) = tf32_small(v, b);
             }
             fence_proxy_async();
-            bar_arrive(bar_full + 8 * stage);
-            return true;
-        };
-        if constexpr (!FUSED) {
-            float4 va[8], vb[8], na[8], nb[8];
-            load(p.dpre, 128, 32, 0, va);
-            load(p.x, p.Din, nfB, 0, vb);
-            for (int64_t blk = 0; blk < nblk; ++blk) {
-                load(p.dpre, 128, 32, blk + 1, na);
-                load(p.x, p.Din, nfB, blk + 1, nb);
-                if (!stage_in(blk, va, vb)) break;
-#pragma unroll
-                for (int q = 0; q < 8; ++q) { va[q] = na[q]; vb[q] = nb[q]; }
-            }
-        } else if constexpr (MASK) {
-            float4 va[8], vb[8], na[8];
-            uint2 nm[4];
-            auto load_mask = [&](int64_t blk) {
-#pragma unroll
-                for (int q = 0; q < 4; ++q) {
-                    const int64_t r = r_begin + blk * 32 + rl + 8 * q;
-                    nm[q] = (blk < nblk && r < r_end) ? __ldg(reinterpret_cast<const uint2*>(p.mask + (size_t)r * 4) + (fl & 1))
-                                                      : make_uint2(0u, 0u);
-                }
-            };
-            auto promote = [&]() {
-#pragma unroll
-                for (int q = 0; q < 8; ++q) {
-                    const uint2 m = nm[q & 3];
-                    const int s = 4 * (warp + 4 * (q >> 2)) + 2 * (fl >> 1);
-                    va[q].x = (m.x >> s) & 1u ? na[q].x : 0.f; va[q].y = (m.x >> (s + 1)) & 1u ? na[q].y : 0.f;
-                    va[q].z = (m.y >> s) & 1u ? na[q].z : 0.f; va[q].w = (m.y >> (s + 1)) & 1u ? na[q].w : 0.f;
-                }
-            };
-            load(p.dpre, 128, 32, 0, na);
-            load_mask(0);
-            promote();
-            for (int64_t blk = 0; blk < nblk; ++blk) {
-                if (tid == 0 && blk + L2_AHEAD < nblk) {
-                    const int64_t ra = r_begin + 32 * (blk + L2_AHEAD), nr = (r_end - ra < 32) ? r_end - ra : 32;
-                    prefetch_l2(p.dpre + (size_t)ra * 128, (uint32_t)(nr * 512));
-                    prefetch_l2(p.x + (size_t)ra * p.Din, (uint32_t)(nr * p.Din * 4));
-                }
-                load(p.dpre, 128, 32, blk + 1, na);
-                load_mask(blk + 1);
-                load(p.x, p.Din, nfB, blk, vb);
-                if (!stage_in(blk, va, vb)) break;
-                promote();
-            }
-        } else {
-            float4 va[8], vb[8], na[8], nm[8];
-            auto promote = [&]() {
-#pragma unroll
-                for (int q = 0; q < 8; ++q) {
-                    va[q] = na[q];
-                    if (p.act) {
-                        va[q].x = nm[q].x > 0.f ? va[q].x : 0.f; va[q].y = nm[q].y > 0.f ? va[q].y : 0.f;
-                        va[q].z = nm[q].z > 0.f ? va[q].z : 0.f; va[q].w = nm[q].w > 0.f ? va[q].w : 0.f;
+            __syncwarp();
+            if (lane == 0) { bar_arrive(bar_bfull + 8 * slot); bar_arrive(bar_empty + 8 * stage); }
+            if (++stage == ns) { stage = 0; phase ^= 1; }
+        }
+        if (tid == 0) ring_drain(bar_full, ns, i_stage, i_phase, i_blk);
+    } else {
+        asm volatile("setmaxnreg.inc.sync.aligned.u32 %0;" ::"n"(CONSUMER_REGS));
+        const int wg = (warp - PRODUCERS / 32) >> 2, g = lane >> 2, t = lane & 3;
+        const int i0 = wg * 64 + (warp & 3) * 16 + g;
+        const int mword = (i0 >> 1) & 3, mbit = 2 * (i0 >> 3) + (i0 & 1);
+        float acc[64] = {}, sum[64];
+        uint32_t ab0[16], as0[16], ab1[16], as1[16];
+#pragma unroll
+        for (int i = 0; i < 64; ++i) sum[i] = 0.f;
+        int stage = 0;
+        uint32_t phase = 0;
+        int64_t blk = 0;
+        bool alive = true;
+        auto step = [&](uint32_t* ab, uint32_t* as) {
+            const int slot = (int)(blk & 1);
+            if (!bar_wait(bar_full + 8 * stage, phase, p.err)) { alive = false; return; }
+            const unsigned char* st = smem + stage * stage_bytes;
+#pragma unroll
+            for (int j = 0; j < 4; ++j) {
+#pragma unroll
+                for (int kh = 0; kh < 2; ++kh) {
+                    const int r = 8 * j + t + 4 * kh;
+                    uint32_t m = 0;
+                    if constexpr (DPRE == 1) m = *reinterpret_cast<const uint32_t*>(st + mask_at + r * 16 + mword * 4);
+#pragma unroll
+                    for (int h = 0; h < 2; ++h) {
+                        const int e = h + 2 * kh;
+                        const int off = box_off(r, i0 + 8 * h);
+                        float v = *reinterpret_cast<const float*>(st + off);
+                        if constexpr (DPRE == 1) v = (m >> (mbit + 2 * h)) & 1u ? v : 0.f;
+                        if constexpr (DPRE == 2) {
+                            if (with_y) v = *reinterpret_cast<const float*>(st + 4 * BOX_BYTES + off) > 0.f ? v : 0.f;
+                        }
+                        const float b = tf32_big(v);
+                        ab[4 * j + e] = __float_as_uint(b);
+                        as[4 * j + e] = __float_as_uint(tf32_small(v, b));
                     }
                 }
-            };
-            load(p.dpre, 128, 32, 0, na);
-            if (p.act) load(p.act, 128, 32, 0, nm);
-            promote();
-            for (int64_t blk = 0; blk < nblk; ++blk) {
-                if (tid == 0 && blk + L2_AHEAD < nblk) {
-                    const int64_t ra = r_begin + 32 * (blk + L2_AHEAD), nr = (r_end - ra < 32) ? r_end - ra : 32;
-                    prefetch_l2(p.dpre + (size_t)ra * 128, (uint32_t)(nr * 512));
-                    if (p.act) prefetch_l2(p.act + (size_t)ra * 128, (uint32_t)(nr * 512));
-                    prefetch_l2(p.x + (size_t)ra * p.Din, (uint32_t)(nr * p.Din * 4));
-                }
-                load(p.dpre, 128, 32, blk + 1, na);
-                if (p.act) load(p.act, 128, 32, blk + 1, nm);
-                load(p.x, p.Din, nfB, blk, vb);
-                if (!stage_in(blk, va, vb)) break;
-                promote();
-            }
-        }
-    } else {
-        const int wg = (warp - PRODUCERS / 32) >> 2;
-        float acc[64] = {}, sum[64];
-#pragma unroll
-        for (int i = 0; i < 64; ++i) sum[i] = 0.f;
-        for (int64_t blk = 0; blk < nblk; ++blk) {
-            const int stage = (int)(blk % WSTAGE);
-            if (!bar_wait(bar_full + 8 * stage, (uint32_t)((blk / WSTAGE) & 1), p.err)) break;
-            const uint32_t a_big = sbase + stage * STAGE_BYTES + wg * 64 * 128, a_small = a_big + KBLK_BYTES;
-            const uint32_t b_big = sbase + stage * STAGE_BYTES + 2 * KBLK_BYTES, b_small = b_big + KBLK_BYTES;
-            mma_kblock(acc, acc, a_big, a_small, b_big, b_small, (blk % FLUSH) == 0);
+            }
+            __syncwarp();
             if (lane == 0) bar_arrive(bar_empty + 8 * stage);
+            if (!bar_wait(bar_bfull + 8 * slot, (uint32_t)((blk >> 1) & 1), p.err)) { alive = false; return; }
+            const uint32_t b_big = sbase + SMEM_BIMG + slot * 2 * KBLK_BYTES;
+            fence_acc(acc);
+            mma_kblock_rs(acc, acc, ab, as, b_big, b_big + KBLK_BYTES, (blk % FLUSH) == 0);
+            wgmma_wait_1();
+            if (lane == 0 && blk > 0) bar_arrive(bar_bempty + 8 * (slot ^ 1));
             if ((blk % FLUSH) == FLUSH - 1 || blk == nblk - 1) {
+                wgmma_wait_all();
+                fence_acc(acc);
 #pragma unroll
                 for (int i = 0; i < 64; ++i) sum[i] += acc[i];
             }
-        }
+            if (++stage == ns) { stage = 0; phase ^= 1; }
+            ++blk;
+        };
+        while (alive && blk < nblk) {
+            step(ab0, as0);
+            if (alive && blk < nblk) step(ab1, as1);
+        }
+        wgmma_wait_all();
+        if (!alive) return;
         const int w4 = warp & 3;
-        const int i0 = wg * 64 + w4 * 16 + (lane >> 2);
+        const int i1 = wg * 64 + w4 * 16 + (lane >> 2);
 #pragma unroll
         for (int j = 0; j < BN / 8; ++j) {
             const int c = 8 * j + 2 * (lane & 3);
             if (c >= p.Din) continue;
 #pragma unroll
             for (int h = 0; h < 2; ++h) {
-                float* prow = p.partial + ((size_t)blockIdx.x * 128 + i0 + 8 * h) * p.Din;
+                float* prow = p.partial + ((size_t)blockIdx.x * 128 + i1 + 8 * h) * p.Din;
                 *reinterpret_cast<float2*>(prow + c) = make_float2(sum[4 * j + 2 * h], sum[4 * j + 2 * h + 1]);
             }
         }
     }
 }
 
-__global__ void __launch_bounds__(THREADS, 1) dw_tf32x3_kernel(const ParamsW p) { dw_body<false>(p); }
-__global__ void __launch_bounds__(THREADS, 1) linear_bwd_dw_kernel(const ParamsW p) { dw_body<true>(p); }
-__global__ void __launch_bounds__(THREADS, 1) linear_bwd_dw_mask_kernel(const ParamsW p) { dw_body<true, true>(p); }
+#define GNNB_DW_PARAMS const ParamsW p, const __grid_constant__ CUtensorMap tm_dy, const __grid_constant__ CUtensorMap tm_y, \
+                       const __grid_constant__ CUtensorMap tm_x
+__global__ void __launch_bounds__(THREADS, 1) dw_tf32x3_kernel(GNNB_DW_PARAMS) { dw_body<0>(p, &tm_dy, &tm_y, &tm_x); }
+__global__ void __launch_bounds__(THREADS, 1) linear_bwd_dw_kernel(GNNB_DW_PARAMS) { dw_body<2>(p, &tm_dy, &tm_y, &tm_x); }
+__global__ void __launch_bounds__(THREADS, 1) linear_bwd_dw_mask_kernel(GNNB_DW_PARAMS) { dw_body<1>(p, &tm_dy, &tm_y, &tm_x); }
+#undef GNNB_DW_PARAMS
 
 __global__ void dw_reduce_kernel(const float* __restrict__ partial, int nparts, int n, float* __restrict__ dW,
                                  const float* __restrict__ colsum = nullptr, int ncolsum = 0, float* __restrict__ db = nullptr) {
@@ -723,6 +798,30 @@
 }
 static int linear_launch(const float* x, const float* W, int64_t ldw, const float* bias, const float* addend, int relu,
                          int64_t M, int64_t K, int64_t Nout, float* y, uint32_t* mask, cudaStream_t st);
+
+static int kblock_map(CUtensorMap* m, const float* base, int64_t rows, int64_t cols, int64_t ld, int box_rows = tc::BM) {
+    static const PFN_cuTensorMapEncodeTiled_v12000 encode = [] {
+        void* fn = nullptr;
+        cudaDriverEntryPointQueryResult q;
+        if (cudaGetDriverEntryPointByVersion("cuTensorMapEncodeTiled", &fn, 12000, cudaEnableDefault, &q) != cudaSuccess ||
+            q != cudaDriverEntryPointSuccess)
+            fn = nullptr;
+        return reinterpret_cast<PFN_cuTensorMapEncodeTiled_v12000>(fn);
+    }();
+    if (!encode) GNNB_FAIL(GNNB_ECUDA, "the driver does not provide cuTensorMapEncodeTiled");
+    int dev = 0;
+    GNNB_CUDA(cudaGetDevice(&dev));
+    GNNB_CUDA(cudaSetDevice(dev));
+    const cuuint64_t dims[2] = {(cuuint64_t)cols, (cuuint64_t)rows};
+    const cuuint64_t strides[1] = {(cuuint64_t)ld * sizeof(float)};
+    const cuuint32_t box[2] = {(cuuint32_t)tc::BK, (cuuint32_t)box_rows}, estride[2] = {1, 1};
+    const CUresult r = encode(m, CU_TENSOR_MAP_DATA_TYPE_FLOAT32, 2, const_cast<float*>(base), dims, strides, box, estride,
+                              CU_TENSOR_MAP_INTERLEAVE_NONE, CU_TENSOR_MAP_SWIZZLE_128B, CU_TENSOR_MAP_L2_PROMOTION_L2_256B,
+                              CU_TENSOR_MAP_FLOAT_OOB_FILL_NONE);
+    if (r != CUDA_SUCCESS) GNNB_FAIL(GNNB_ECUDA, "cuTensorMapEncodeTiled failed (CUresult %d)", (int)r);
+    return GNNB_OK;
+}
+constexpr int64_t RING_MAX_ROWS = (int64_t)INT32_MAX - tc::BM;
 int linear_tf32x3_ex(const float* x, const float* W, int64_t ldw, const float* bias, const float* addend, int relu, int64_t M,
                      int64_t K, int64_t Nout, float* y, cudaStream_t st) {
     return linear_launch(x, W, ldw, bias, addend, relu, M, K, Nout, y, nullptr, st);
@@ -738,7 +837,7 @@
     const bool wide = K > 128 || Nout > 128;
     if (wide) {
         if (K % 32 != 0 || K > 2048 || Nout % 128 != 0 || Nout > tcx::MAX_NOUT || ldw % 4 != 0 || ldw < K || M < 2048) return GNNB_EUNSUPPORTED;
-    } else if (K % 32 != 0 || Nout % 16 != 0 || Nout < 16 || ldw % 4 != 0 || ldw < K) {
+    } else if (K % 32 != 0 || Nout % 16 != 0 || Nout < 16 || ldw % 4 != 0 || ldw < K || M > RING_MAX_ROWS) {
         return GNNB_EUNSUPPORTED;
     }
     if (((uintptr_t)x & 15) || ((uintptr_t)W & 15) || ((uintptr_t)y & 15) || ((uintptr_t)addend & 15)) return GNNB_EUNSUPPORTED;
@@ -757,16 +856,21 @@
     const int nsm = s->nsm;
     const int64_t ntiles = ceil_div(M, tc::BM);
     const unsigned grid = (unsigned)(ntiles < nsm ? ntiles : nsm);
-    if (wide) tcx::linear_wide_tf32x3_kernel<<<grid, tc::THREADS, tcx::SMEM_TOTAL_X, st>>>(p);
-    else if (mask) tc::linear_relu_mask_kernel<<<grid, tc::THREADS, tc::SMEM_TOTAL, st>>>(p);
-    else tc::linear_tf32x3_kernel<<<grid, tc::THREADS, tc::SMEM_TOTAL, st>>>(p);
+    if (wide) {
+        tcx::linear_wide_tf32x3_kernel<<<grid, tc::THREADS, tcx::SMEM_TOTAL_X, st>>>(p);
+    } else {
+        CUtensorMap tm_x;
+        GNNB_TRY(kblock_map(&tm_x, x, M, K, K));
+        if (mask) tc::linear_relu_mask_kernel<<<grid, tc::THREADS, tc::SMEM_TOTAL, st>>>(p, tm_x);
+        else tc::linear_tf32x3_kernel<<<grid, tc::THREADS, tc::SMEM_TOTAL, st>>>(p, tm_x);
+    }
     GNNB_LAUNCHED();
     return GNNB_OK;
 }
 
 int dw_tf32x3(const float* dpre, const float* x, int64_t M, int64_t Din, int64_t Dout, float* dW, cudaStream_t st) {
     if (!g_tc_enabled) return GNNB_EUNSUPPORTED;
-    if (Dout != 128 || Din % 32 != 0 || Din > 128 || Din < 32) return GNNB_EUNSUPPORTED;
+    if (Dout != 128 || Din % 32 != 0 || Din > 128 || Din < 32 || M > RING_MAX_ROWS) return GNNB_EUNSUPPORTED;
     if (((uintptr_t)dpre & 15) || ((uintptr_t)x & 15) || ((uintptr_t)dW & 15)) return GNNB_EUNSUPPORTED;
     DeviceState* s = nullptr;
     GNNB_TRY(device_state(&s));
@@ -780,7 +884,10 @@
     rpc = ceil_div(rpc, 32) * 32;
     p.rows_per_cta = rpc;
     const int grid = (int)ceil_div(M, rpc);
-    tcw::dw_tf32x3_kernel<<<grid, tc::THREADS, tcw::SMEM_TOTALW, st>>>(p);
+    CUtensorMap tm_dy, tm_x;
+    GNNB_TRY(kblock_map(&tm_dy, dpre, M, 128, 128, 32));
+    GNNB_TRY(kblock_map(&tm_x, x, M, Din, Din, 32));
+    tcw::dw_tf32x3_kernel<<<grid, tc::THREADS, tcw::SMEM_TOTALW, st>>>(p, tm_dy, tm_dy, tm_x);
     GNNB_LAUNCHED();
     const int n = (int)(128 * Din);
     tcw::dw_reduce_kernel<<<(unsigned)ceil_div(n, 256), 256, 0, st>>>(partial, grid, n, dW);
@@ -791,7 +898,7 @@
 int linear_bwd_tf32x3(const float* dy, const float* y, const uint32_t* mask, const float* x, const float* W, int64_t M,
                       int64_t Din, float* dx, float* dW, float* db, cudaStream_t st) {
     if (!g_tc_enabled) return GNNB_EUNSUPPORTED;
-    if (Din % 32 != 0 || Din > 128 || Din < 32 || M <= 0) return GNNB_EUNSUPPORTED;
+    if (Din % 32 != 0 || Din > 128 || Din < 32 || M <= 0 || M > RING_MAX_ROWS) return GNNB_EUNSUPPORTED;
     if (((uintptr_t)dy & 15) || ((uintptr_t)y & 15) || ((uintptr_t)x & 15) || ((uintptr_t)dx & 15) || ((uintptr_t)mask & 15))
         return GNNB_EUNSUPPORTED;
     DeviceState* s = nullptr;
@@ -806,16 +913,23 @@
     p.mask = const_cast<uint32_t*>(mask);
     const int64_t ntiles = ceil_div(M, tc::BM);
     const int grid_dx = (int)(ntiles < nsm ? ntiles : nsm);
-    if (mask) tc::linear_bwd_dx_mask_kernel<<<grid_dx, tc::THREADS, tc::SMEM_TOTAL, st>>>(p);
-    else tc::linear_bwd_dx_kernel<<<grid_dx, tc::THREADS, tc::SMEM_TOTAL, st>>>(p);
+    CUtensorMap tm_dy, tm_y;
+    GNNB_TRY(kblock_map(&tm_dy, dy, M, 128, 128));
+    GNNB_TRY(kblock_map(&tm_y, (y && !mask) ? y : dy, M, 128, 128));
+    if (mask) tc::linear_bwd_dx_mask_kernel<<<grid_dx, tc::THREADS, tc::SMEM_TOTAL, st>>>(p, tm_dy, tm_y);
+    else tc::linear_bwd_dx_kernel<<<grid_dx, tc::THREADS, tc::SMEM_TOTAL, st>>>(p, tm_dy, tm_y);
     GNNB_LAUNCHED();
     tcw::ParamsW pw;
     pw.dpre = dy; pw.x = x; pw.partial = partial; pw.M = M; pw.Din = (int)Din; pw.err = s->tc_err; pw.act = y; pw.mask = mask;
     const int64_t rpc = ceil_div(ceil_div(M, nsm), 32) * 32;
     pw.rows_per_cta = rpc;
     const int grid_dw = (int)ceil_div(M, rpc);
-    if (mask) tcw::linear_bwd_dw_mask_kernel<<<grid_dw, tc::THREADS, tcw::SMEM_TOTALW, st>>>(pw);
-    else tcw::linear_bwd_dw_kernel<<<grid_dw, tc::THREADS, tcw::SMEM_TOTALW, st>>>(pw);
+    CUtensorMap tw_dy, tw_y, tw_x;
+    GNNB_TRY(kblock_map(&tw_dy, dy, M, 128, 128, 32));
+    GNNB_TRY(kblock_map(&tw_y, (y && !mask) ? y : dy, M, 128, 128, 32));
+    GNNB_TRY(kblock_map(&tw_x, x, M, Din, Din, 32));
+    if (mask) tcw::linear_bwd_dw_mask_kernel<<<grid_dw, tc::THREADS, tcw::SMEM_TOTALW, st>>>(pw, tw_dy, tw_y, tw_x);
+    else tcw::linear_bwd_dw_kernel<<<grid_dw, tc::THREADS, tcw::SMEM_TOTALW, st>>>(pw, tw_dy, tw_y, tw_x);
     GNNB_LAUNCHED();
     const int n = (int)(128 * Din);
     tcw::dw_reduce_kernel<<<(unsigned)ceil_div(n + 128, 256), 256, 0, st>>>(partial, grid_dw, n, dW, colsum, grid_dx * 4, db);
diff --git a/graphneuralnetworks.jl_b200/csrc/tma.cuh b/graphneuralnetworks.jl_b200/csrc/tma.cuh
--- a/graphneuralnetworks.jl_b200/csrc/tma.cuh
+++ b/graphneuralnetworks.jl_b200/csrc/tma.cuh
@@ -31,6 +31,10 @@
     asm volatile("cp.async.bulk.shared::cluster.global.mbarrier::complete_tx::bytes [%0], [%1], %2, [%3];"
                  ::"r"(dst), "l"(src), "r"(bytes), "r"(bar) : "memory");
 }
+__device__ __forceinline__ void tensor_load_2d(uint32_t dst, const void* map, int x0, int x1, uint32_t bar) {
+    asm volatile("cp.async.bulk.tensor.2d.shared::cluster.global.tile.mbarrier::complete_tx::bytes [%0], [%1, {%2, %3}], [%4];"
+                 ::"r"(dst), "l"(map), "r"(x0), "r"(x1), "r"(bar) : "memory");
+}
 
 }
 }
```

Result: faster. 2.433 billion, median of 6 (+6.8%).
